# gorgonia/agogo

Hardware: AMD Instinct MI355X
Metric: mcts_sims_per_sec (higher is better)
Workload: dtype f32 (Winograd F(5x5,3x3): fp32 transforms; transform-domain products as fp16x2 = each fp32 operand scaled by a power of two and split into 2 fp16 pieces (22-23 significand bits, absolute error <= 2^-38 of the tensor range), 3 fp16 MFMAs per product, fp32 accumulate)

## Files before the change

agogo_amd/capi.py:

```python
import ctypes as C
import os

import numpy as np

_HERE = os.path.dirname(os.path.abspath(__file__))
_LIB = None

NONE, BLACK, WHITE = 0, 1, 2
PASS, RESIGN = -1, -2
NO_MOVE = -32768
GAME_MNK, GAME_C4, GAME_KOMI, GAME_WQ = 0, 1, 2, 3
ENC_TWOPLANE, ENC_WQ = 0, 1
INF_NET, INF_DUMMY, INF_SCRIPT, INF_HASH, INF_UNIFORM, INF_CALLBACK = 0, 1, 2, 3, 4, 5
BN_DEGENERATE_EPS, BN_RUNNING, BN_IDENTITY = 0, 1, 2
COMPUTE_F32_MFMA, COMPUTE_BF16X3, COMPUTE_FP16X2, COMPUTE_WINO, COMPUTE_AUTO, COMPUTE_WINO_H2 = 0, 1, 2, 3, 4, 5
COMPUTE_FORCE = 0x100
PROF_CONV, PROF_HEADS, PROF_SELECT, PROF_EXPAND, PROF_MOVE, PROF_CONV_INIT = 0, 1, 2, 3, 4, 5
PROF_WINO_IN, PROF_WINO_GEMM, PROF_WINO_OUT = 6, 7, 8
DONT_PREFER_PASS, PREFER_PASS, DONT_RESIGN = 0, 1, 2
POOL_STRICT, POOL_STOP_SEARCH, POOL_GROW = 0, 1, 2


class AgzError(RuntimeError):
    pass
# ... 59 lines not shown

    def tramp(_user, bp):
        try:
            b = bp.contents
            n, F, H, W, pl = b.n, b.features, b.height, b.width, b.policy_len
            as_np = np.ctypeslib.as_array
            leaves = {"planes": as_np(b.planes, shape=(n, F, H, W)), "board": as_np(b.board, shape=(n, H * W)),
                      "to_move": as_np(b.to_move, shape=(n,)), "move_number": as_np(b.move_number, shape=(n,)),
                      "game": as_np(b.game, shape=(n,)), "policy_len": pl}
            pol, val = py(leaves)
            as_np(b.policy, shape=(n, pl))[...] = np.asarray(pol, np.float32).reshape(n, pl)
            as_np(b.value, shape=(n,))[...] = np.asarray(val, np.float32).reshape(n)
            return 0
        except BaseException as e:
            box["exc"] = e
            return 1

    fn = INFER_FN(tramp)
    fn._box = box
    return fn


def lib_path():
    return os.environ.get("AGZ_LIB_PATH") or os.path.join(_HERE, "lib", "libagz.so")


def lib():
    global _LIB
    if _LIB is not None:
        return _LIB
    path = lib_path()
    if not os.path.exists(path):
        raise AgzError("libagz.so not built (%s): run `make` or __graft_entry__.build(); there is no CPU fallback"
                       % path)
    L = C.CDLL(path)
    vp, i32, u64, f64 = C.c_void_p, C.c_int, C.c_uint64, C.c_double
    pvp = C.POINTER(C.c_void_p)
    pf, pi, pu, pu8 = C.POINTER(C.c_float), C.POINTER(C.c_int32), C.POINTER(C.c_uint32), C.POINTER(C.c_uint8)

    def sig(name, res, *args):
        f = getattr(L, name)
        f.restype = res
        f.argtypes = list(args)

    sig("agz_last_error", C.c_char_p)
    sig("agz_version", C.c_char_p)
    sig("agz_ctx_create", i32, i32, pvp)
    sig("agz_ctx_destroy", None, vp)
    sig("agz_ctx_sync", i32, vp)
    sig("agz_ctx_stream", vp, vp)
    sig("agz_ctx_prof_enable", i32, vp, i32)
    sig("agz_ctx_prof_read", i32, vp, i32, C.POINTER(C.c_int64), C.POINTER(C.c_double))
    sig("agz_net_create", i32, vp, C.POINTER(NetConf), pvp)
    sig("agz_net_destroy", None, vp)
    sig("agz_net_num_params", i32, vp)
    sig("agz_net_param_info", i32, vp, i32, C.c_char_p, C.c_size_t, C.POINTER(C.c_size_t))
    sig("agz_net_set_param", i32, vp, i32, pf, C.c_size_t)
    sig("agz_net_get_param", i32, vp, i32, pf, C.c_size_t)
    sig("agz_net_set_bn_stats", i32, vp, i32, pf, pf, C.c_size_t)
    sig("agz_net_init_random", i32, vp, u64)
    sig("agz_net_commit", i32, vp)
    sig("agz_net_infer", i32, vp, pf, i32, pf, pf)
    sig("agz_net_infer_dev", i32, vp, vp, i32, vp, vp)
    sig("agz_host_alloc", i32, vp, C.c_size_t, pvp)
    sig("agz_host_free", i32, vp, vp)
    sig("agz_mcts_to_dot", i32, vp, i32, C.c_char_p, C.c_size_t, C.POINTER(C.c_size_t))
    sig("agz_mcts_set_timeout_ms", i32, vp, i32)
    sig("agz_mcts_last_simulations", i32, vp, C.POINTER(C.c_int64))
    sig("agz_net_set_latency_mode", i32, vp, i32)
    sig("agz_net_set_tower_queues", i32, vp, i32)
    sig("agz_net_set_compute_mode", i32, vp, i32)
    sig("agz_net_flops_per_eval", f64, vp)
    sig("agz_net_save", i32, vp, C.c_char_p)
    sig("agz_net_load", i32, vp, C.c_char_p)
    sig("agz_arena_get_results", i32, vp, C.POINTER(C.c_int64), C.POINTER(C.c_int64), C.POINTER(C.c_int64))
    sig("agz_trainer_create", i32, vp, C.POINTER(NetConf), pvp)
    sig("agz_trainer_create_tied", i32, vp, C.POINTER(NetConf), pvp)
    sig("agz_trainer_is_tied", i32, vp, C.POINTER(i32))
    sig("agz_trainer_destroy", None, vp)
    sig("agz_trainer_num_params", i32, vp)
    sig("agz_trainer_param_info", i32, vp, i32, C.c_char_p, C.c_size_t, C.POINTER(C.c_size_t))
    sig("agz_trainer_set_param", i32, vp, i32, pf, C.c_size_t)
    sig("agz_trainer_get_param", i32, vp, i32, pf, C.c_size_t)
    sig("agz_trainer_get_grad", i32, vp, i32, pf, C.c_size_t)
    sig("agz_trainer_init_random", i32, vp, u64)
    sig("agz_trainer_batch", i32, vp, pf, pf, pf, C.c_float, pf)
    sig("agz_trainer_forward_backward", i32, vp, pf, pf, pf, pf)
    sig("agz_trainer_forward_backward_dev", i32, vp, vp, vp, vp, pf)
    sig("agz_trainer_apply", i32, vp, C.c_float, C.c_float)
    sig("agz_trainer_grads_dev", i32, vp, pvp, C.POINTER(C.c_size_t))
    sig("agz_trainer_set_solver", i32, vp, C.POINTER(SolverConf))
    sig("agz_trainer_get_solver", i32, vp, C.POINTER(SolverConf))
    sig("agz_trainer_get_velocity", i32, vp, i32, pf, C.c_size_t)
    sig("agz_trainer_set_velocity", i32, vp, i32, pf, C.c_size_t)
    sig("agz_trainer_reset_solver", i32, vp)
    sig("agz_trainer_set_adam", i32, vp, C.POINTER(AdamConf))
    sig("agz_trainer_get_adam", i32, vp, C.POINTER(AdamConf), C.POINTER(C.c_uint64))
    sig("agz_trainer_get_moments", i32, vp, i32, pf, pf, C.c_size_t)
    sig("agz_trainer_set_moments", i32, vp, i32, pf, pf, C.c_size_t)
    sig("agz_trainer_set_bn_tracking", i32, vp, i32, C.c_float)
    sig("agz_trainer_get_bn_tracking", i32, vp, C.POINTER(C.c_int), C.POINTER(C.c_float), C.POINTER(C.c_double))
    sig("agz_trainer_num_bn", i32, vp)
    sig("agz_trainer_get_bn_stats", i32, vp, i32, pf, pf, C.c_size_t)
    sig("agz_trainer_set_bn_stats", i32, vp, i32, pf, pf, C.c_size_t, C.c_double)
    sig("agz_trainer_reset_bn_stats", i32, vp)
    sig("agz_trainer_eval", i32, vp, pf, pf, pf, pf)
    sig("agz_trainer_eval_dev", i32, vp, vp, vp, vp, pf)
    sig("agz_trainer_set_compute_mode", i32, vp, i32)
    sig("agz_train", i32, vp, pf, pf, pf, i32, i32, u64, pf)
    sig("agz_trainer_export", i32, vp, vp)
    sig("agz_trainer_save", i32, vp, C.c_char_p)
    sig("agz_trainer_load", i32, vp, C.c_char_p)
    sig("agz_arena_create", i32, vp, C.POINTER(GameConf), C.POINTER(MctsConf), i32, u64, i32, pvp)
    sig("agz_arena_destroy", None, vp)
    sig("agz_arena_set_inferencer", i32, vp, i32, i32, vp)
    sig("agz_arena_reset", i32, vp, pu8)
    sig("agz_arena_play", i32, vp, i32, i32)
    sig("agz_arena_selfplay", i32, vp, C.c_int64, i32)
    sig("agz_arena_set_parallel", i32, vp, i32)
    sig("agz_arena_begin_move", i32, vp)
    sig("agz_arena_simulate", i32, vp, i32)
    sig("agz_arena_end_move", i32, vp, i32)
    sig("agz_arena_apply_moves", i32, vp, pi)
    sig("agz_arena_get_stats", i32, vp, C.POINTER(ArenaStats))
    sig("agz_arena_get_game", i32, vp, i32, pi, C.POINTER(GameState))
    sig("agz_arena_get_history", i32, vp, i32, pi, i32, pi)
    sig("agz_arena_root_children", i32, vp, i32, i32, pi, pu, pf, pf, i32, pi)
    sig("agz_arena_tree_nodes", i32, vp, i32, i32, pi)
    sig("agz_arena_get_examples", i32, vp, pf, pf, pf, pi, i32, pi)
    sig("agz_arena_clear_examples", i32, vp)
    sig("agz_arena_drop_labelled_examples", i32, vp)
    sig("agz_arena_examples_dev", i32, vp, pvp, pvp, pvp, pi)
    i64, pi64 = C.c_int64, C.POINTER(C.c_int64)
    sig("agz_train_dev", i32, vp, vp, vp, vp, i32, i32, u64, pf)
    sig("agz_examples_create", i32, vp, i32, i32, i32, i32, pvp)
    sig("agz_examples_destroy", None, vp)
    sig("agz_examples_count", i32, vp, pi64)
    sig("agz_examples_clear", i32, vp)
    sig("agz_examples_append_arena", i32, vp, vp)
    sig("agz_examples_append_dev", i32, vp, vp, vp, vp, i64)
    sig("agz_examples_append_host", i32, vp, pf, pf, pf, i64)
    sig("agz_examples_get", i32, vp, pf, pf, pf, i64, pi64)
    sig("agz_examples_augment_rotate", i32, vp)
    sig("agz_examples_prepare", i32, vp, i32, i32, u64, pi)
    sig("agz_examples_tensors_dev", i32, vp, pvp, pvp, pvp, pi64, pi)
    sig("agz_examples_get_tensors", i32, vp, pf, pf, pf)
    sig("agz_examples_raw_dev", i32, vp, pvp, pvp, pvp)
    sig("agz_rotate_boards", i32, vp, pf, i32, i32, i32, pf)
    sig("agz_ctx_prof_set_stride", i32, vp, i32, i32)
    sig("agz_wino_stages", i32, vp, pf, pf, i32, i32, i32, i32, i32, pf, pf)
    sig("agz_wino_h2_tile", i32, i32, i32)
    sig("agz_net_set_wino_h2_form", i32, vp, i32)
    sig("agz_net_set_wino_h2_gemm", i32, vp, i32)
    sig("agz_net_min_same_batch", i32, vp, i32, i32, C.POINTER(C.c_int))
    sig("agz_arena_set_prep_compact", i32, vp, i32)
    sig("agz_arena_set_split", i32, vp, i32)
    sig("agz_arena_split_steps", i32, vp, C.POINTER(C.c_int64), C.POINTER(C.c_int64), C.POINTER(C.c_int))
    sig("agz_trainer_set_dma_forward", i32, vp, i32)
    sig("agz_arena_last_prep_batch", i32, vp, C.POINTER(C.c_int), C.POINTER(C.c_int))
    sig("agz_arena_debug_counter", i32, vp, i32, C.POINTER(C.c_int64))
    sig("agz_arena_pool_capacity", i32, vp, C.POINTER(C.c_int), C.POINTER(C.c_int))
    sig("agz_wino_h2_chained", i32, i32, i32, i32)
    sig("agz_arena_random_moves", i32, vp, pi, u64)
    sig("agz_arena_set_state", i32, vp, i32, C.POINTER(State))
    sig("agz_arena_examples_labelled_dev", i32, vp, pvp)
    sig("agz_mcts_create", i32, vp, C.POINTER(GameConf), C.POINTER(MctsConf), u64, i32, pvp)
    sig("agz_mcts_destroy", None, vp)
    sig("agz_mcts_set_inferencer", i32, vp, i32, vp)
    sig("agz_mcts_set_inferencer_callback", i32, vp, INFER_FN, vp, i32)
    sig("agz_arena_set_inferencer_callback", i32, vp, i32, INFER_FN, vp, i32)
    sig("agz_arena_set_pool_policy", i32, vp, i32)
    sig("agz_mcts_set_pool_policy", i32, vp, i32)
    sig("agz_mcts_set_parallel", i32, vp, i32)
    sig("agz_mcts_set_game", i32, vp, C.POINTER(State))
    sig("agz_mcts_search", i32, vp, i32, pi)
    sig("agz_mcts_policies", i32, vp, pf, i32)
    sig("agz_mcts_root_children", i32, vp, pi, pu, pf, pf, i32, pi)
    sig("agz_mcts_nodes", i32, vp, pi)
    sig("agz_mcts_children", i32, vp, i32, pi, pi, pu, pf, pf, i32, pi)
    sig("agz_mcts_get_stats", i32, vp, C.POINTER(ArenaStats))
    sig("agz_mcts_reset", i32, vp)
    sig("agz_comm_init_all", i32, pvp, i32, pvp)
    sig("agz_comm_unique_id", i32, vp)
    sig("agz_comm_init_rank", i32, vp, i32, i32, vp, pvp)
    sig("agz_comm_destroy", None, vp)
    sig("agz_comm_rank", i32, vp)
    sig("agz_comm_size", i32, vp)
    sig("agz_examples_allgather", i32, vp, vp)
    sig("agz_trainer_allreduce", i32, vp, vp)
    sig("agz_trainer_forward_backward_allreduce", i32, vp, vp, pf, pf, pf, pf)
    sig("agz_trainer_forward_backward_allreduce_dev", i32, vp, vp, vp, vp, vp, pf)
    sig("agz_comm_debug_fail_slice", i32, vp, i32)
    sig("agz_trainer_create_sharded", i32, vp, C.POINTER(NetConf), pvp)
    sig("agz_trainer_create_sharded_tied", i32, vp, C.POINTER(NetConf), pvp)
    sig("agz_trainer_shard", i32, vp, C.POINTER(i32), C.POINTER(i32), C.POINTER(i32))
    sig("agz_comm_debug_fail_layer", i32, vp, i32)
    _LIB = L
    return L


def _check(r, what=""):
    if r != 0:
        raise AgzError("%s failed (%d): %s" % (what, r, lib().agz_last_error().decode(errors="replace")))


def _pf(a):
    return a.ctypes.data_as(C.POINTER(C.c_float))


def _pi(a):
    return a.ctypes.data_as(C.POINTER(C.c_int32))


class Ctx:
    def __init__(self, device=0):
        self.h = C.c_void_p()
        self._children = []
        _check(lib().agz_ctx_create(device, C.byref(self.h)), "agz_ctx_create")

    def _adopt(self, child):
        import weakref
        self._children.append(weakref.ref(child))

    def close(self):
        if self.h:
            kids = [r() for r in self._children]
            for k in sorted([k for k in kids if k is not None], key=lambda k: 0 if isinstance(k, Arena) else 1):
                k.close()
            self._children = []
            for p in list(getattr(self, "_pinned", {}).values()):
                lib().agz_host_free(self.h, C.c_void_p(p))
            self._pinned = {}
            lib().agz_ctx_destroy(self.h)
            self.h = C.c_void_p()

    def __del__(self):
        try:
            self.close()
        except Exception:
            pass

    def host_array(self, shape, dtype=np.float32):
        n = int(np.prod(shape)) * np.dtype(dtype).itemsize
        p = C.c_void_p()
        _check(lib().agz_host_alloc(self.h, max(n, 1), C.byref(p)), "agz_host_alloc")
        arr = np.ctypeslib.as_array((C.c_char * max(n, 1)).from_address(p.value)).view(dtype)[: int(np.prod(shape))].reshape(shape)
        self._pinned = getattr(self, "_pinned", {})
        self._pinned[arr.ctypes.data] = p.value
        return arr

    def host_free(self, arr):
        p = getattr(self, "_pinned", {}).pop(arr.ctypes.data, None)
        if p is not None and self.h:
            _check(lib().agz_host_free(self.h, C.c_void_p(p)), "agz_host_free")

    def sync(self):
        _check(lib().agz_ctx_sync(self.h), "agz_ctx_sync")

    def stream(self):
        return lib().agz_ctx_stream(self.h)

    def prof_enable(self, on=True, classes=None):
        if on and classes is not None:
            mask = 0
            for k in classes:
                mask |= 1 << (k + 1)
            _check(lib().agz_ctx_prof_enable(self.h, mask), "agz_ctx_prof_enable")
            return
        return self._prof_enable_all(on)

    def prof_set_stride(self, klass, stride):
        _check(lib().agz_ctx_prof_set_stride(self.h, int(klass), int(stride)), "agz_ctx_prof_set_stride")

    def _prof_enable_all(self, on=True):
        _check(lib().agz_ctx_prof_enable(self.h, int(on)), "agz_ctx_prof_enable")

    def prof_read(self, klass):
        n, ms = C.c_int64(0), C.c_double(0)
        _check(lib().agz_ctx_prof_read(self.h, klass, C.byref(n), C.byref(ms)), "agz_ctx_prof_read")
        return n.value, ms.value


class Net:

    def __init__(self, ctx, K, SharedLayers, FC, Width, Height, Features, ActionSpace, BatchSize=256,
                 bn_mode=BN_DEGENERATE_EPS, bn_eps=1e-5):
        self.ctx = ctx
        self.conf = NetConf(K, SharedLayers, FC, BatchSize, Width, Height, Features, ActionSpace, bn_mode, bn_eps)
        self.h = C.c_void_p()
        _check(lib().agz_net_create(ctx.h, C.byref(self.conf), C.byref(self.h)), "agz_net_create")
        ctx._adopt(self)

    def close(self):
        if self.h and self.ctx.h:
            lib().agz_net_destroy(self.h)
        self.h = C.c_void_p()

    def __del__(self):
        try:
            self.close()
        except Exception:
            pass

    def num_params(self):
        return lib().agz_net_num_params(self.h)

    def param_info(self, i):
        name = C.create_string_buffer(128)
        n = C.c_size_t(0)
        _check(lib().agz_net_param_info(self.h, i, name, 128, C.byref(n)), "agz_net_param_info")
        return name.value.decode(), n.value

    def set_param(self, i, v):
        a = np.ascontiguousarray(v, dtype=np.float32).ravel()
        _check(lib().agz_net_set_param(self.h, i, _pf(a), a.size), "agz_net_set_param")

    def get_param(self, i):
        _, n = self.param_info(i)
        a = np.zeros(n, dtype=np.float32)
        _check(lib().agz_net_get_param(self.h, i, _pf(a), a.size), "agz_net_get_param")
        return a

    def set_bn_stats(self, bi, mean, var):
        m = np.ascontiguousarray(mean, dtype=np.float32)
        v = np.ascontiguousarray(var, dtype=np.float32)
        _check(lib().agz_net_set_bn_stats(self.h, bi, _pf(m), _pf(v), m.size), "agz_net_set_bn_stats")

    def init_random(self, seed):
        _check(lib().agz_net_init_random(self.h, seed), "agz_net_init_random")

    def commit(self):
        _check(lib().agz_net_commit(self.h), "agz_net_commit")

    def infer(self, planes):
        c = self.conf
        x = np.ascontiguousarray(planes, dtype=np.float32).reshape(-1, c.Features, c.Height, c.Width)
        B = x.shape[0]
        pol = np.zeros((B, c.ActionSpace), dtype=np.float32)
        val = np.zeros(B, dtype=np.float32)
        _check(lib().agz_net_infer(self.h, _pf(x), B, _pf(pol), _pf(val)), "agz_net_infer")
        return pol, val

    def set_compute_mode(self, mode):
        _check(lib().agz_net_set_compute_mode(self.h, int(mode)), "agz_net_set_compute_mode")

    def set_latency_mode(self, on=True):
        _check(lib().agz_net_set_latency_mode(self.h, int(on)), "agz_net_set_latency_mode")

    def set_tower_queues(self, queues):
        _check(lib().agz_net_set_tower_queues(self.h, int(queues)), "agz_net_set_tower_queues")

    def set_wino_h2_form(self, form):
        _check(lib().agz_net_set_wino_h2_form(self.h, int(form)), "agz_net_set_wino_h2_form")

    def set_wino_h2_gemm(self, variant):
        _check(lib().agz_net_set_wino_h2_gemm(self.h, int(variant)), "agz_net_set_wino_h2_gemm")

    def min_same_batch(self, n, G):
        b = C.c_int(0)
        _check(lib().agz_net_min_same_batch(self.h, int(n), int(G), C.byref(b)), "agz_net_min_same_batch")
        return b.value

    def infer_dev(self, planes_ptr, B, policy_ptr, value_ptr):
        _check(lib().agz_net_infer_dev(self.h, C.c_void_p(planes_ptr), B, C.c_void_p(policy_ptr),
                                       C.c_void_p(value_ptr)), "agz_net_infer_dev")

    def flops_per_eval(self):
        return lib().agz_net_flops_per_eval(self.h)

    def save(self, path):
        _check(lib().agz_net_save(self.h, os.fsencode(path)), "agz_net_save")

    def load(self, path):
        _check(lib().agz_net_load(self.h, os.fsencode(path)), "agz_net_load")


class Trainer:

    def __init__(self, ctx, K, SharedLayers, FC, Width, Height, Features, ActionSpace, BatchSize, bn_eps=1e-5, tied=False):
        self.ctx = ctx
        self.conf = NetConf(K, SharedLayers, FC, BatchSize, Width, Height, Features, ActionSpace, 0, bn_eps)
        self.h = C.c_void_p()
        if tied:
            _check(lib().agz_trainer_create_tied(ctx.h, C.byref(self.conf), C.byref(self.h)), "agz_trainer_create_tied")
        else:
            _check(lib().agz_trainer_create(ctx.h, C.byref(self.conf), C.byref(self.h)), "agz_trainer_create")
        ctx._adopt(self)

    def is_tied(self):
        v = C.c_int(0)
        _check(lib().agz_trainer_is_tied(self.h, C.byref(v)), "agz_trainer_is_tied")
        return bool(v.value)

    @classmethod
    def sharded(cls, ctx, comm, K, SharedLayers, FC, Width, Height, Features, ActionSpace, BatchSize, bn_eps=1e-5, tied=False):
        assert comm.ctx is ctx, "the communicator belongs to another context"
        self = cls.__new__(cls)
        self.ctx, self.comm = ctx, comm
        self.conf = NetConf(K, SharedLayers, FC, BatchSize, Width, Height, Features, ActionSpace, 0, bn_eps)
        self.h = C.c_void_p()
        if tied:
            _check(lib().agz_trainer_create_sharded_tied(comm.h, C.byref(self.conf), C.byref(self.h)), "agz_trainer_create_sharded_tied")
        else:
            _check(lib().agz_trainer_create_sharded(comm.h, C.byref(self.conf), C.byref(self.h)), "agz_trainer_create_sharded")
        ctx._adopt(self)
        return self

    def shard(self):
        r0, n, nr = C.c_int(0), C.c_int(0), C.c_int(0)
        _check(lib().agz_trainer_shard(self.h, C.byref(r0), C.byref(n), C.byref(nr)), "agz_trainer_shard")
        return r0.value, n.value, nr.value

    def close(self):
        if self.h and self.ctx.h:
            lib().agz_trainer_destroy(self.h)
        self.h = C.c_void_p()

    def __del__(self):
        try:
            self.close()
        except Exception:
            pass

    def num_params(self):
        return lib().agz_trainer_num_params(self.h)

    def param_info(self, i):
        name = C.create_string_buffer(128)
        n = C.c_size_t(0)
        _check(lib().agz_trainer_param_info(self.h, i, name, 128, C.byref(n)), "agz_trainer_param_info")
        return name.value.decode(), n.value

    def set_param(self, i, v):
        a = np.ascontiguousarray(v, dtype=np.float32).ravel()
        _check(lib().agz_trainer_set_param(self.h, i, _pf(a), a.size), "agz_trainer_set_param")

    def get_param(self, i):
        a = np.zeros(self.param_info(i)[1], np.float32)
        _check(lib().agz_trainer_get_param(self.h, i, _pf(a), a.size), "agz_trainer_get_param")
        return a

    def get_grad(self, i):
        a = np.zeros(self.param_info(i)[1], np.float32)
        _check(lib().agz_trainer_get_grad(self.h, i, _pf(a), a.size), "agz_trainer_get_grad")
        return a

    def init_random(self, seed):
        _check(lib().agz_trainer_init_random(self.h, seed), "agz_trainer_init_random")

    def batch(self, planes, pi, v, lr=0.1):
        x = np.ascontiguousarray(planes, np.float32)
        p = np.ascontiguousarray(pi, np.float32)
        vv = np.ascontiguousarray(v, np.float32)
        c = C.c_float(0)
        _check(lib().agz_trainer_batch(self.h, _pf(x), _pf(p), _pf(vv), lr, C.byref(c)), "agz_trainer_batch")
        return c.value

    def forward_backward(self, planes, pi, v):
        x = np.ascontiguousarray(planes, np.float32)
        p = np.ascontiguousarray(pi, np.float32)
        vv = np.ascontiguousarray(v, np.float32)
        c = C.c_float(0)
        _check(lib().agz_trainer_forward_backward(self.h, _pf(x), _pf(p), _pf(vv), C.byref(c)), "agz_trainer_forward_backward")
        return c.value

    def forward_backward_dev(self, planes_ptr, pi_ptr, v_ptr, want_cost=True):
        c = C.c_float(0)
        _check(lib().agz_trainer_forward_backward_dev(self.h, C.c_void_p(planes_ptr), C.c_void_p(pi_ptr), C.c_void_p(v_ptr),
                                                      C.byref(c) if want_cost else None), "agz_trainer_forward_backward_dev")
        return c.value if want_cost else None

    def apply(self, lr=0.1, grad_scale=1.0):
        _check(lib().agz_trainer_apply(self.h, lr, grad_scale), "agz_trainer_apply")

    def set_solver(self, momentum=0.0, l2reg=0.0, clip=0.0, reserved=0):
        sc = SolverConf(momentum, l2reg, clip, reserved)
        _check(lib().agz_trainer_set_solver(self.h, C.byref(sc)), "agz_trainer_set_solver")

    def get_solver(self):
        sc = SolverConf()
        _check(lib().agz_trainer_get_solver(self.h, C.byref(sc)), "agz_trainer_get_solver")
        return {"momentum": sc.momentum, "l2reg": sc.l2reg, "clip": sc.clip}

    def get_velocity(self, i):
        a = np.zeros(self.param_info(i)[1], np.float32)
        _check(lib().agz_trainer_get_velocity(self.h, i, _pf(a), a.size), "agz_trainer_get_velocity")
        return a

    def set_velocity(self, i, v):
        a = np.ascontiguousarray(v, dtype=np.float32).ravel()
        _check(lib().agz_trainer_set_velocity(self.h, i, _pf(a), a.size), "agz_trainer_set_velocity")

    def reset_solver(self):
        _check(lib().agz_trainer_reset_solver(self.h), "agz_trainer_reset_solver")

    def set_adam(self, beta1=0.9, beta2=0.999, eps=1e-8, on=True):
        ac = AdamConf(beta1, beta2, eps, int(on))
        _check(lib().agz_trainer_set_adam(self.h, C.byref(ac)), "agz_trainer_set_adam")

    def get_adam(self):
        ac, t = AdamConf(), C.c_uint64(0)
        _check(lib().agz_trainer_get_adam(self.h, C.byref(ac), C.byref(t)), "agz_trainer_get_adam")
        return {"beta1": ac.beta1, "beta2": ac.beta2, "eps": ac.eps, "on": bool(ac.on), "t": int(t.value)}

    def get_moments(self, i):
        m = np.zeros(self.param_info(i)[1], np.float32)
        v = np.zeros_like(m)
        _check(lib().agz_trainer_get_moments(self.h, i, _pf(m), _pf(v), m.size), "agz_trainer_get_moments")
        return m, v

# ... 561 lines not shown
```

agogo_amd/csrc/conv_wino_h2.hpp:

```cpp
#pragma once

template <int TM> struct WinoT;
template <> struct WinoT<4> {
  static constexpr int AL = 6, VSHIFT = 7;
  static constexpr float BT[6][6] = {{4, 0, -5, 0, 1, 0}, {0, -4, -4, 1, 1, 0}, {0, 4, -4, -1, 1, 0}, {0, -2, -1, 2, 1, 0}, {0, 2, -1, -2, 1, 0}, {0, 4, 0, -5, 0, 1}};
  static constexpr float AT[4][6] = {{1, 1, 1, 1, 1, 0}, {0, 1, -1, 2, -2, 0}, {0, 1, 1, 4, 4, 0}, {0, 1, -1, 8, -8, 1}};
  static constexpr double G[6][3] = {{1.0 / 4, 0, 0}, {-1.0 / 6, -1.0 / 6, -1.0 / 6}, {-1.0 / 6, 1.0 / 6, -1.0 / 6}, {1.0 / 24, 1.0 / 12, 1.0 / 6}, {1.0 / 24, -1.0 / 12, 1.0 / 6}, {0, 0, 1}};
};
template <> struct WinoT<5> {
  static constexpr int AL = 7, VSHIFT = 6;
  static constexpr float BT[7][7] = {{-0.5f, 0.25f, 2.5f, -1.25f, -2, 1, 0}, {0, 0.5f, 0.25f, -2.25f, -1, 1, 0}, {0, -0.5f, 0.75f, 1.75f, -3, 1, 0},
                                     {0, 1, 1.5f, -2, -1.5f, 1, 0},          {0, -1, 2.5f, 0, -2.5f, 1, 0},       {0, 0.25f, 0, -1.25f, 0, 1, 0},
                                     {0, -0.5f, 0.25f, 2.5f, -1.25f, -2, 1}};
  static constexpr float AT[5][7] = {{1, 1, 1, 1, 1, 1, 0}, {0, 1, -1, 0.5f, -0.5f, 2, 0}, {0, 1, 1, 0.25f, 0.25f, 4, 0}, {0, 1, -1, 0.125f, -0.125f, 8, 0},
                                     {0, 1, 1, 0.0625f, 0.0625f, 16, 1}};
  static constexpr double G[7][3] = {{-2, 0, 0}, {-2.0 / 3, -2.0 / 3, -2.0 / 3}, {-2.0 / 9, 2.0 / 9, -2.0 / 9}, {16.0 / 9, 8.0 / 9, 4.0 / 9}, {16.0 / 15, -8.0 / 15, 4.0 / 15},
                                     {2.0 / 45, 4.0 / 45, 8.0 / 45}, {0, 0, 1}};
};
template <int TM> __device__ __forceinline__ void wino_btv(const float* d, float* o);
template <int TM> __device__ __forceinline__ void wino_atv(const float* m, float* o);
template <> __device__ __forceinline__ void wino_btv<4>(const float* d, float* o) { wino_bt6(d, o); }
template <> __device__ __forceinline__ void wino_atv<4>(const float* m, float* o) { wino_at4(m, o); }
template <> __device__ __forceinline__ void wino_btv<5>(const float* d, float* o) {
  o[0] = -0.5f * d[0] + 0.25f * d[1] + 2.5f * d[2] - 1.25f * d[3] - 2.f * d[4] + d[5];
  o[1] = 0.5f * d[1] + 0.25f * d[2] - 2.25f * d[3] - d[4] + d[5];
  o[2] = -0.5f * d[1] + 0.75f * d[2] + 1.75f * d[3] - 3.f * d[4] + d[5];
  o[3] = d[1] + 1.5f * d[2] - 2.f * d[3] - 1.5f * d[4] + d[5];
  o[4] = -d[1] + 2.5f * (d[2] - d[4]) + d[5];
  o[5] = 0.25f * d[1] - 1.25f * d[3] + d[5];
  o[6] = -0.5f * d[1] + 0.25f * d[2] + 2.5f * d[3] - 1.25f * d[4] - 2.f * d[5] + d[6];
}
template <> __device__ __forceinline__ void wino_atv<5>(const float* m, float* o) {
  const float s12 = m[1] + m[2], d12 = m[1] - m[2], s34 = m[3] + m[4], d34 = m[3] - m[4];
  o[0] = m[0] + s12 + s34 + m[5];
  o[1] = d12 + 0.5f * d34 + 2.f * m[5];
  o[2] = s12 + 0.25f * s34 + 4.f * m[5];
  o[3] = d12 + 0.125f * d34 + 8.f * m[5];
  o[4] = s12 + 0.0625f * s34 + 16.f * m[5] + m[6];
}

typedef unsigned u32x2_t __attribute__((ext_vector_type(2)));
struct WinoH2Args;
__device__ __forceinline__ size_t h2_row(const WinoH2Args& h, int pos, int t);
struct WinoH2Args {
  WinoArgs w;
  int tm, npos;
  int rsh, rmask;
  unsigned rA, rB;
  int raw;
  const float* w_unscale_dev;
  int fuse_prev;
  int wm_per_board;
  unsigned* amax_self;
  int in_swap;
  const _Float16* U2;
  const unsigned* amax_in;
  unsigned* amax_out;
  float* wave_max;
  float w_unscale;
  const float* t_in;
  const float* col_unscale;
  const float* t_next;
  int cform;
  const _Float16* U2c;
  const float* amax_true;
  const float* wm_prev;
  float* wm_out;
  unsigned* amax_next;
  float g1, g0;
  int gemm_variant;
  int temporal_stores;
  int row_pad;
};
__device__ __forceinline__ size_t h2_row(const WinoH2Args& h, int pos, int t) {
  return (size_t)(t >> h.rsh) * h.rA + (size_t)pos * h.rB + (size_t)(t & h.rmask);
}

__device__ __forceinline__ void wino_h2_scales(unsigned amax_bits, int shift, float* s, float* inv) {
  int e = (int)((amax_bits >> 23) & 0xffu);
  if (amax_bits == 0u) { *s = 1.f; *inv = 1.f; return; }
  e = e < 30 ? 30 : (e > 230 ? 230 : e);
  *s = __uint_as_float((unsigned)(268 - shift - e) << 23);
  *inv = __uint_as_float((unsigned)(e - 14 + shift) << 23);
}

__device__ __forceinline__ unsigned wino_h2_pack(float a, float b, unsigned* lo) {
  const _Float16 ha = (_Float16)a, hb = (_Float16)b;
  const _Float16 la = (_Float16)(a - (float)ha), lb = (_Float16)(b - (float)hb);
  *lo = (unsigned)__builtin_bit_cast(unsigned short, la) | ((unsigned)__builtin_bit_cast(unsigned short, lb) << 16);
  return (unsigned)__builtin_bit_cast(unsigned short, ha) | ((unsigned)__builtin_bit_cast(unsigned short, hb) << 16);
}

template <int TM>
__global__ __launch_bounds__(256) void wino_in_h2_kernel(WinoH2Args h) {
  using WT = WinoT<TM>;
  constexpr int AL = WT::AL;
  const WinoArgs& a = h.w;
  const int C2 = a.C >> 1;
  const size_t g = (size_t)blockIdx.x * 256 + threadIdx.x;
  if (g >= (size_t)a.T * C2) return;
  const int c2 = (int)(g % C2);
  const int t = (int)(g / C2);
  const int b = t / a.TPB, tt = t - b * a.TPB;
  const int ty = tt / a.ntx, tx = tt - ty * a.ntx;
  unsigned amax_bits;
  if (h.fuse_prev) {
    const float* wp = h.wave_max + (size_t)b * h.wm_per_board;
    float mx = 0.f;
    for (int i = threadIdx.x & 63; i < h.wm_per_board; i += 64) mx = fmaxf(mx, wp[i]);
#pragma unroll
    for (int o = 32; o > 0; o >>= 1) mx = fmaxf(mx, __shfl_xor(mx, o, 64));
    amax_bits = __float_as_uint(mx);
    if (tt == 0 && c2 == 0) h.amax_self[b] = amax_bits;
  } else {
    amax_bits = h.amax_in[b];
  }
  float sb, inv_;
  wino_h2_scales(amax_bits, WT::VSHIFT, &sb, &inv_);
  float sbx = sb, sby = sb;
  if (h.t_in) { const float2 t2 = *reinterpret_cast<const float2*>(h.t_in + 2 * c2); sbx *= t2.x; sby *= t2.y; }
  const float* xb = a.x + (size_t)b * a.Hp * a.Wp * a.C + 2 * c2;
  float2 d[AL][AL];
#pragma unroll
  for (int j = 0; j < AL; j++) {
    const int px = TM * tx + j, pxc = px < a.Wp ? px : a.Wp - 1;
#pragma unroll
    for (int i = 0; i < AL; i++) {
      const int py = TM * ty + i, pyc = py < a.Hp ? py : a.Hp - 1;
      d[i][j] = *reinterpret_cast<const float2*>(xb + ((size_t)pyc * a.Wp + pxc) * a.C);
    }
  }
  float tmx[AL][AL], tmy[AL][AL];
#pragma unroll
  for (int j = 0; j < AL; j++) {
    const bool okx = TM * tx + j < a.Wp;
    float dx[AL], dy[AL], ox[AL], oy[AL];
#pragma unroll
    for (int i = 0; i < AL; i++) {
      const bool ok = okx && TM * ty + i < a.Hp;
      dx[i] = ok ? d[i][j].x : 0.f; dy[i] = ok ? d[i][j].y : 0.f;
    }
    wino_btv<TM>(dx, ox);
    wino_btv<TM>(dy, oy);
#pragma unroll
    for (int i = 0; i < AL; i++) { tmx[i][j] = ox[i]; tmy[i][j] = oy[i]; }
  }
  unsigned* V2 = reinterpret_cast<unsigned*>(a.V);
  const int c = 2 * c2;
  const size_t word_in_row = (size_t)(c >> 5) * 32 + ((c & 31) >> 1);
  const int lane = threadIdx.x & 63;
  const size_t swap_word = (size_t)((c2 >> 6) * 4) * 32 + lane;
#pragma unroll
  for (int i = 0; i < AL; i++) {
    float ox[AL], oy[AL];
    wino_btv<TM>(tmx[i], ox);
    wino_btv<TM>(tmy[i], oy);
#pragma unroll
    for (int j = 0; j < AL; j++) {
      unsigned lo;
      const unsigned hi = wino_h2_pack(ox[j] * sbx, oy[j] * sby, &lo);
      if (h.cform) {
        const auto s16 = __builtin_amdgcn_permlane16_swap(hi, lo, false, false);
        const unsigned e0 = s16[0], e1 = s16[1];
        const int NS = a.C >> 5;
        const size_t chunk0 = ((size_t)(t >> 7) * h.npos + (size_t)(i * AL + j)) * NS + (size_t)((c2 >> 6) * 4 + 2 * (lane >> 5));
        unsigned* p0 = V2 + chunk0 * 4096 + (size_t)(t & 127) * 32 + (lane & 31);
        p0[0] = e0;
        p0[4096] = e1;
        continue;
      }
      unsigned* rowp = V2 + h2_row(h, i * AL + j, t) * a.C;
      if (h.in_swap) {
        const auto s16 = __builtin_amdgcn_permlane16_swap(hi, lo, false, false);
        const unsigned e0 = s16[0], e1 = s16[1];
        const auto s32 = __builtin_amdgcn_permlane32_swap(e0, e1, false, false);
        const unsigned w0 = s32[0], w1 = s32[1];
        rowp[swap_word] = w0;
        rowp[swap_word + 64] = w1;
      } else {
        rowp[word_in_row] = hi;
        rowp[word_in_row + 16] = lo;
      }
    }
  }
}

__global__ __launch_bounds__(256, 3) void wino_gemm_h2_kernel(WinoH2Args h) {
  const WinoArgs& a = h.w;
  constexpr int PIECE = 128 * 64;
  constexpr int STAGE = 4 * PIECE;
  __shared__ __attribute__((aligned(16))) unsigned char lds[STAGE];

  const int per_pos = a.n_mtiles * a.n_ntiles;
  const int nblk = h.npos * per_pos;
  const int id = blockIdx.x;
  int q = nblk >> 3, rr = nblk & 7, xcd = id & 7, slot = id >> 3;
  int tile = (xcd < rr ? xcd * (q + 1) : rr * (q + 1) + (xcd - rr) * q) + slot;
  const int pos = tile / per_pos;
  const int rem = tile - pos * per_pos;
  const int m_tile = rem / a.n_ntiles, n_tile = rem - m_tile * a.n_ntiles;
  const int m0 = m_tile * 128, n0 = n_tile * 128;

  const int tid = threadIdx.x, lane = tid & 63, wid = tid >> 6;
  const int wm = wid >> 1, wn = wid & 1;
  const int srow = tid >> 1, shalf = tid & 1;
  int mrow = m0 + srow;
  if (mrow >= a.T) mrow = a.T - 1;
  int nrow = n0 + srow;
  if (nrow >= a.Ntot) nrow = a.Ntot - 1;
  const int NK = a.C >> 5;
  const unsigned piece_bytes = (unsigned)a.Ntot * 64u;
  unsigned xo_ = (unsigned)((h2_row(h, pos, mrow) * a.C) * 4) + (unsigned)shalf * 32u;
  unsigned wo_ = (unsigned)pos * (unsigned)NK * 2u * piece_bytes + (unsigned)nrow * 64u + (unsigned)shalf * 32u;
  const unsigned s_off0 = h2_lds_off(srow, 2 * shalf), s_off1 = h2_lds_off(srow, 2 * shalf + 1);

  f32x16 acc[2][2];
#pragma unroll
  for (int i = 0; i < 2; i++)
#pragma unroll
    for (int j = 0; j < 2; j++)
#pragma unroll
      for (int r = 0; r < 16; r++) acc[i][j][r] = 0.f;

  int ra[2], rb[2];
#pragma unroll
  for (int i = 0; i < 2; i++) ra[i] = (wm * 2 + i) * 32 + (lane & 31);
#pragma unroll
  for (int j = 0; j < 2; j++) rb[j] = (wn * 2 + j) * 32 + (lane & 31);
  const int kh = lane >> 5;

  u32x4_t xa0, xa1, xa2, xa3, xb0, xb1, xb2, xb3;
  const char* xbase = reinterpret_cast<const char*>(a.V);
  const char* wbase = reinterpret_cast<const char*>(h.U2);
  int f_n = 0;
#define WH2_GLOAD()                                                                           \
  xa0 = *reinterpret_cast<const u32x4_t*>(xbase + xo_);                                       \
  xa1 = *reinterpret_cast<const u32x4_t*>(xbase + xo_ + 16u);                                 \
  xa2 = *reinterpret_cast<const u32x4_t*>(xbase + xo_ + 64u);                                 \
  xa3 = *reinterpret_cast<const u32x4_t*>(xbase + xo_ + 80u);                                 \
  xb0 = *reinterpret_cast<const u32x4_t*>(wbase + wo_);                                       \
  xb1 = *reinterpret_cast<const u32x4_t*>(wbase + wo_ + 16u);                                 \
  xb2 = *reinterpret_cast<const u32x4_t*>(wbase + wo_ + piece_bytes);                         \
  xb3 = *reinterpret_cast<const u32x4_t*>(wbase + wo_ + piece_bytes + 16u);                   \
  if (f_n + 1 < NK) { f_n++; xo_ += 128u; wo_ += 2u * piece_bytes; }
#define WH2_STORE()                                                                           \
  *reinterpret_cast<u32x4_t*>(lds + 0 * PIECE + s_off0) = xa0;                                \
  *reinterpret_cast<u32x4_t*>(lds + 0 * PIECE + s_off1) = xa1;                                \
  *reinterpret_cast<u32x4_t*>(lds + 1 * PIECE + s_off0) = xa2;                                \
  *reinterpret_cast<u32x4_t*>(lds + 1 * PIECE + s_off1) = xa3;                                \
  *reinterpret_cast<u32x4_t*>(lds + 2 * PIECE + s_off0) = xb0;                                \
  *reinterpret_cast<u32x4_t*>(lds + 2 * PIECE + s_off1) = xb1;                                \
  *reinterpret_cast<u32x4_t*>(lds + 3 * PIECE + s_off0) = xb2;                                \
  *reinterpret_cast<u32x4_t*>(lds + 3 * PIECE + s_off1) = xb3;
#define WH2_QUAD(PA_, PB_)                                                                    \
  _Pragma("unroll") for (int i = 0; i < 2; i++)                                               \
    _Pragma("unroll") for (int j = 0; j < 2; j++)                                             \
      acc[i][j] = __builtin_amdgcn_mfma_f32_32x32x16_f16(A_[i][PA_], B_[j][PB_], acc[i][j], 0, 0, 0);

  WH2_GLOAD()
  for (int it = 0; it < NK; it++) {
    WH2_STORE()
    __syncthreads();
    WH2_GLOAD()
#pragma unroll
    for (int ks = 0; ks < 2; ks++) {
      f16x8_t A_[2][2], B_[2][2];
#pragma unroll
      for (int p = 0; p < 2; p++) {
#pragma unroll
        for (int i = 0; i < 2; i++) A_[i][p] = *reinterpret_cast<const f16x8_t*>(lds + p * PIECE + h2_lds_off(ra[i], 2 * ks + kh));
#pragma unroll
        for (int j = 0; j < 2; j++) B_[j][p] = *reinterpret_cast<const f16x8_t*>(lds + (2 + p) * PIECE + h2_lds_off(rb[j], 2 * ks + kh));
      }
      WH2_QUAD(1, 0) WH2_QUAD(0, 1) WH2_QUAD(0, 0)
    }
    __syncthreads();
  }
#undef WH2_QUAD
#undef WH2_STORE
#undef WH2_GLOAD

#pragma unroll
  for (int i = 0; i < 2; i++) {
#pragma unroll
    for (int r = 0; r < 16; r++) {
      const int row = (wm * 2 + i) * 32 + (r & 3) + 8 * (r >> 2) + 4 * (lane >> 5);
      const int m = m0 + row;
      if (m < a.T) {
        float* dst = a.Mb + h2_row(h, pos, m) * a.Ntot;
#pragma unroll
        for (int j = 0; j < 2; j++) {
          const int c = n0 + (wn * 2 + j) * 32 + (lane & 31);
          if (c < a.Ntot) dst[c] = acc[i][j][r];
        }
      }
    }
  }
}

__global__ __launch_bounds__(256, 2) void wino_gemm_h2w_kernel(WinoH2Args h) {
  const WinoArgs& a = h.w;
  constexpr int PA = 128 * 64, PB = 256 * 64;
  constexpr int STAGE = 2 * PA + 2 * PB;
  __shared__ __attribute__((aligned(16))) unsigned char lds[STAGE];

  const int n_nt = (a.Ntot + 255) / 256;
  const int per_pos = a.n_mtiles * n_nt;
  const int nblk = h.npos * per_pos;
  const int id = blockIdx.x;
  int q = nblk >> 3, rr = nblk & 7, xcd = id & 7, slot = id >> 3;
  int tile = (xcd < rr ? xcd * (q + 1) : rr * (q + 1) + (xcd - rr) * q) + slot;
  const int pos = tile / per_pos;
  const int rem = tile - pos * per_pos;
  const int m_tile = rem / n_nt, n_tile = rem - m_tile * n_nt;
  const int m0 = m_tile * 128, n0 = n_tile * 256;

  const int tid = threadIdx.x, lane = tid & 63, wid = tid >> 6;
  const int wm = wid >> 1, wn = wid & 1;
  const int srow = tid >> 1, shalf = tid & 1;
// ... 832 lines not shown
```

agogo_amd/csrc/conv_wino_h2c.hpp:

```cpp
#pragma once

__device__ __forceinline__ unsigned h2c_img(int row, int slot) { return maps::h2c_img(row, slot); }

template <int NK, int PFA>
__global__ __launch_bounds__(256, 2) void wino_gemm_h2c_kernel(WinoH2Args h) {
  const WinoArgs& a = h.w;
  constexpr int SA = 128 * 128, SB = 256 * 128;
  __shared__ __attribute__((aligned(16))) unsigned char lds[SA + SB];

  const int n_nt = a.Ntot >> 8;
  const int per_pos = a.n_mtiles * n_nt;
  const int nblk = h.npos * per_pos;
  const int id = blockIdx.x;
  int q = nblk >> 3, rr = nblk & 7, xcd = id & 7, slot = id >> 3;
  int tile = (xcd < rr ? xcd * (q + 1) : rr * (q + 1) + (xcd - rr) * q) + slot;
  const int pos = tile / per_pos;
  const int rem = tile - pos * per_pos;
  const int m_tile = rem / n_nt, n_tile = rem - m_tile * n_nt;

  const int tid = threadIdx.x, lane = tid & 63, wid = tid >> 6;
  const int wm = wid >> 1, wn = wid & 1;
  const unsigned st_lds = h2c_img(tid >> 3, tid & 7);
  const char* abase = reinterpret_cast<const char*>(a.V) + ((size_t)m_tile * h.npos + pos) * (size_t)NK * SA + (size_t)tid * 16;
  const char* bbase = reinterpret_cast<const char*>(h.U2c) + (((size_t)pos * NK) * n_nt + n_tile) * (size_t)SB + (size_t)tid * 16;
  const size_t bstep = (size_t)n_nt * SB;

  f32x16 acc[2][4];
#pragma unroll
  for (int i = 0; i < 2; i++)
#pragma unroll
    for (int j = 0; j < 4; j++)
#pragma unroll
      for (int r = 0; r < 16; r++) acc[i][j][r] = 0.f;

  const int kh = lane >> 5, sw = (lane >> 1) & 7;
  const unsigned fa = (unsigned)((wm * 64 + (lane & 31)) * 128);
  const unsigned fb = (unsigned)(SA + (wn * 128 + (lane & 31)) * 128);

  u32x4_t xa[PFA][4], xb[8];
  auto load_a = [&](int set, int kk) {
#pragma unroll
    for (int j = 0; j < 4; j++) xa[set][j] = *reinterpret_cast<const u32x4_t*>(abase + (size_t)kk * SA + j * 4096);
  };
  auto load_b = [&](int kk) {
#pragma unroll
    for (int j = 0; j < 8; j++) xb[j] = *reinterpret_cast<const u32x4_t*>(bbase + (size_t)kk * bstep + j * 4096);
  };
  load_b(0);
#pragma unroll
  for (int p = 0; p < PFA; p++) load_a(p, p < NK ? p : NK - 1);
#pragma unroll
  for (int it = 0; it < NK; it++) {
    const int set = it % PFA;
#pragma unroll
    for (int j = 0; j < 4; j++) *reinterpret_cast<u32x4_t*>(lds + st_lds + j * 4096) = xa[set][j];
#pragma unroll
    for (int j = 0; j < 8; j++) *reinterpret_cast<u32x4_t*>(lds + SA + st_lds + j * 4096) = xb[j];
    __syncthreads();
    if (it + 1 < NK) load_b(it + 1);
    if (it + PFA < NK) load_a(set, it + PFA);
#pragma unroll
    for (int ks = 0; ks < 2; ks++) {
      f16x8_t A_[2][2], B_[4][2];
#pragma unroll
      for (int p = 0; p < 2; p++) {
        const unsigned so = (unsigned)(((p * 4 + 2 * ks + kh) ^ sw) << 4);
#pragma unroll
        for (int i = 0; i < 2; i++) A_[i][p] = *reinterpret_cast<const f16x8_t*>(lds + fa + i * 4096 + so);
#pragma unroll
        for (int j = 0; j < 4; j++) B_[j][p] = *reinterpret_cast<const f16x8_t*>(lds + fb + j * 4096 + so);
      }
#pragma unroll
      for (int pp = 0; pp < 3; pp++) {
        const int pa = pp == 0 ? 1 : 0, pb = pp == 1 ? 1 : 0;
#pragma unroll
        for (int i = 0; i < 2; i++)
#pragma unroll
          for (int j = 0; j < 4; j++) acc[i][j] = __builtin_amdgcn_mfma_f32_32x32x16_f16(A_[i][pa], B_[j][pb], acc[i][j], 0, 0, 0);
      }
    }
    __syncthreads();
  }

  float* mbase = a.Mb + ((((size_t)m_tile * h.npos + pos) * (size_t)(a.Ntot >> 6) + (size_t)n_tile * 4 + wn * 2) * 128 + (size_t)(wm * 64)) * 64 + lane;
#pragma unroll
  for (int qq = 0; qq < 2; qq++)
#pragma unroll
    for (int i = 0; i < 2; i++)
#pragma unroll
      for (int r = 0; r < 16; r++) {
        const unsigned x0 = __float_as_uint(acc[i][2 * qq][r]), x1 = __float_as_uint(acc[i][2 * qq + 1][r]);
        const auto s32 = __builtin_amdgcn_permlane32_swap(x0, x1, false, false);
        const unsigned w0 = s32[0], w1 = s32[1];
        float* d = mbase + (size_t)qq * 8192 + (size_t)(i * 32 + (r & 3) + 8 * (r >> 2)) * 64;
        d[0] = __uint_as_float(w0);
        d[4 * 64] = __uint_as_float(w1);
      }
}

typedef __attribute__((address_space(3))) void* h2c_lds_ptr_t;
template <int NK, bool NT = true>
__global__ __launch_bounds__(256, 3) void wino_gemm_h2g_kernel(WinoH2Args h) {
  const WinoArgs& a = h.w;
  constexpr int SA = 128 * 128, SB = 256 * 128;
  __shared__ __attribute__((aligned(16))) unsigned char lds[SA + SB];

  const int n_nt = a.Ntot >> 8;
  const int per_pos = a.n_mtiles * n_nt;
  const int nblk = h.npos * per_pos;
  const int id = blockIdx.x;
  int q = nblk >> 3, rr = nblk & 7, xcd = id & 7, slot = id >> 3;
  int tile = (xcd < rr ? xcd * (q + 1) : rr * (q + 1) + (xcd - rr) * q) + slot;
  const int pos = tile / per_pos;
  const int rem = tile - pos * per_pos;
  const int m_tile = rem / n_nt, n_tile = rem - m_tile * n_nt;

  const int tid = threadIdx.x, lane = tid & 63;
  const int wid = __builtin_amdgcn_readfirstlane(tid >> 6);
  const int wm = wid >> 1, wn = wid & 1;
  const __amdgpu_buffer_rsrc_t ar = h2_rsrc(a.V), br = h2_rsrc(h.U2c);
  const unsigned vo_e = maps::h2c_dma_src(lane, 0), vo_o = maps::h2c_dma_src(lane, 1);
  const unsigned a_w = maps::h2c_wave_part(wid, 128), b_w = maps::h2c_wave_part(wid, 256);
  unsigned a_so = (unsigned)(((size_t)m_tile * h.npos + pos) * (size_t)NK * SA) + a_w;
  unsigned b_so = (unsigned)((((size_t)pos * NK) * n_nt + n_tile) * (size_t)SB) + b_w;
  const unsigned b_step = (unsigned)n_nt * SB;
  unsigned char* const la = lds + a_w;
  unsigned char* const lb = lds + SA + b_w;

  f32x16 acc[2][4];
#pragma unroll
  for (int i = 0; i < 2; i++)
#pragma unroll
    for (int j = 0; j < 4; j++)
#pragma unroll
      for (int r = 0; r < 16; r++) acc[i][j][r] = 0.f;

#pragma nounroll
  for (int it = 0; it < NK; it++) {
#pragma unroll
    for (int j = 0; j < maps::h2c_wave_instrs(128); j++)
      __builtin_amdgcn_raw_ptr_buffer_load_lds(ar, (h2c_lds_ptr_t)(la + maps::h2c_dma_dst(0, j)), 16, (j & 1) ? vo_o : vo_e,
                                               a_so + (maps::h2c_dma_src(0, j) - maps::h2c_dma_src(0, j & 1)), 0, 0);
#pragma unroll
    for (int j = 0; j < maps::h2c_wave_instrs(256); j++)
      __builtin_amdgcn_raw_ptr_buffer_load_lds(br, (h2c_lds_ptr_t)(lb + maps::h2c_dma_dst(0, j)), 16, (j & 1) ? vo_o : vo_e,
                                               b_so + (maps::h2c_dma_src(0, j) - maps::h2c_dma_src(0, j & 1)), 0, 0);
    a_so += SA; b_so += b_step;
    __syncthreads();
#pragma unroll
    for (int ks = 0; ks < 2; ks++) {
      f16x8_t A_[2][2];
#pragma unroll
      for (int i = 0; i < 2; i++) {
        A_[i][0] = *reinterpret_cast<const f16x8_t*>(lds + maps::h2c_frag(wm * 64 + i * 32, lane, 0, ks));
        A_[i][1] = *reinterpret_cast<const f16x8_t*>(lds + maps::h2c_frag(wm * 64 + i * 32, lane, 1, ks));
      }
#pragma unroll
      for (int j = 0; j < 4; j++) {
        const f16x8_t b0 = *reinterpret_cast<const f16x8_t*>(lds + SA + maps::h2c_frag(wn * 128 + j * 32, lane, 0, ks));
        const f16x8_t b1 = *reinterpret_cast<const f16x8_t*>(lds + SA + maps::h2c_frag(wn * 128 + j * 32, lane, 1, ks));
#pragma unroll
        for (int i = 0; i < 2; i++) {
          acc[i][j] = __builtin_amdgcn_mfma_f32_32x32x16_f16(A_[i][1], b0, acc[i][j], 0, 0, 0);
          acc[i][j] = __builtin_amdgcn_mfma_f32_32x32x16_f16(A_[i][0], b1, acc[i][j], 0, 0, 0);
          acc[i][j] = __builtin_amdgcn_mfma_f32_32x32x16_f16(A_[i][0], b0, acc[i][j], 0, 0, 0);
        }
      }
    }
    __syncthreads();
  }

  float* mbase = a.Mb + maps::mc_index(m_tile, h.npos, pos, a.Ntot >> 6, n_tile * 4 + wn * 2, wm * 64, lane);
#pragma unroll
  for (int qq = 0; qq < 2; qq++)
#pragma unroll
    for (int i = 0; i < 2; i++)
#pragma unroll
      for (int r = 0; r < 16; r++) {
        const unsigned x0 = __float_as_uint(acc[i][2 * qq][r]), x1 = __float_as_uint(acc[i][2 * qq + 1][r]);
        const auto s32 = __builtin_amdgcn_permlane32_swap(x0, x1, false, false);
        const unsigned w0 = s32[0], w1 = s32[1];
        float* d = mbase + maps::mc_index(0, 0, 0, 0, qq, i * 32 + maps::mfma_row(r), 0);
        if (NT) {
          __builtin_nontemporal_store(__uint_as_float(w0), d);
          __builtin_nontemporal_store(__uint_as_float(w1), d + maps::mc_index(0, 0, 0, 0, 0, 4, 0));
        } else {
          d[0] = __uint_as_float(w0);
          d[maps::mc_index(0, 0, 0, 0, 0, 4, 0)] = __uint_as_float(w1);
        }
      }
}


typedef unsigned h2p_rsrc_t __attribute__((ext_vector_type(4)));
__device__ __forceinline__ void h2p_dma16(h2p_rsrc_t rsrc, unsigned lds_addr, unsigned voff, unsigned soff) {
  unsigned keep;
  asm volatile("s_mov_b32 %0, m0\n\ts_mov_b32 m0, %1\n\ts_nop 0\n\tbuffer_load_dwordx4 %2, %3, %4 offen lds\n\ts_mov_b32 m0, %0"
               : "=&s"(keep) : "s"(lds_addr), "v"(voff), "s"(rsrc), "s"(soff) : "memory");
}
__device__ __forceinline__ void h2p_dma16x2(h2p_rsrc_t rsrc, unsigned lds_a, unsigned lds_b, unsigned voff_a, unsigned voff_b, unsigned soff) {
  unsigned keep;
  asm volatile("s_mov_b32 %0, m0\n\ts_mov_b32 m0, %1\n\ts_nop 0\n\tbuffer_load_dwordx4 %3, %5, %6 offen lds\n\t"
               "s_mov_b32 m0, %2\n\ts_nop 0\n\tbuffer_load_dwordx4 %4, %5, %6 offen lds\n\ts_mov_b32 m0, %0"
               : "=&s"(keep) : "s"(lds_a), "s"(lds_b), "v"(voff_a), "v"(voff_b), "s"(rsrc), "s"(soff) : "memory");
}
#define H2P_WAIT(N) asm volatile("s_waitcnt vmcnt(%0)" ::"n"(N) : "memory")
template <int MODE>
__global__ __launch_bounds__(256, 1) void wino_gemm_h2p_kernel(WinoH2Args h) {
  const WinoArgs& a = h.w;
  constexpr int NK = maps::H2P_NK, R = maps::H2P_R, SA = 64 * 128, D = maps::H2P_D;
  __shared__ __attribute__((aligned(1024))) unsigned char lds[R * SA];

  const int tid = threadIdx.x, lane = tid & 63;
  const int wid = __builtin_amdgcn_readfirstlane(tid >> 6), wm = wid >> 1, wn = wid & 1;
  const int n_slabs = a.Ntot >> 7, n_nt = a.Ntot >> 8;
  const maps::H2pTeam tm = maps::h2p_team((int)blockIdx.x, (int)gridDim.x, n_slabs);
  if (tm.idle) return;
  const int team = tm.team, slab = tm.slab, nteams = tm.nteams;
  const int n_half = a.n_mtiles * 2, U2 = h.npos * a.n_mtiles;
  const int u0 = maps::h2p_u0(team, nteams, U2), nT = maps::h2p_u0(team + 1, nteams, U2) - u0;
  if (nT <= 0) return;

  h2p_rsrc_t ar;
  {
    const unsigned long long u = (unsigned long long)a.V;
    ar[0] = __builtin_amdgcn_readfirstlane((unsigned)u); ar[1] = __builtin_amdgcn_readfirstlane((unsigned)(u >> 32) & 0xffffu);
    ar[2] = 0x7fffffffu; ar[3] = 0x00020000u;
  }
  const unsigned vo_e = maps::h2c_dma_src(lane, 0), vo_o = maps::h2c_dma_src(lane, 1);
  static_assert(maps::h2c_wave_instrs(64) == 2, "two DMA instructions per wave and stage");
  const unsigned a_w = maps::h2c_wave_part(wid, 64);
  const unsigned dma_l = (unsigned)(size_t)(h2c_lds_ptr_t)lds + a_w;
  auto issue = [&](unsigned vb, int kk, int rslot) {
    if (MODE & 2) return;
    const unsigned so = vb + (unsigned)kk * 16384u + a_w;
    h2p_dma16x2(ar, dma_l + (unsigned)rslot * SA + maps::h2c_dma_dst(0, 0), dma_l + (unsigned)rslot * SA + maps::h2c_dma_dst(0, 1), vo_e, vo_o, so);
  };
  const int kh = lane >> 5;
  auto frag = [&](int rslot, int ks, int p) -> f16x8_t {
    return *reinterpret_cast<const f16x8_t*>(lds + rslot * SA + maps::h2c_frag(wm * 32, lane, p, ks));
  };

  f16x8_t Bf[NK][2][2][2];
  auto load_b = [&](int pos) {
    const char* bb = reinterpret_cast<const char*>(h.U2c) + ((size_t)pos * NK * n_nt + (slab >> 1)) * 32768 +
                     (size_t)(((slab & 1) * 128 + wn * 64 + (lane & 31)) * 128 + kh * 16);
#pragma unroll
    for (int kk = 0; kk < NK; kk++)
#pragma unroll
      for (int ks = 0; ks < 2; ks++)
#pragma unroll
        for (int j = 0; j < 2; j++)
#pragma unroll
          for (int p = 0; p < 2; p++)
            Bf[kk][ks][j][p] = *reinterpret_cast<const f16x8_t*>(bb + (size_t)kk * n_nt * 32768 + j * 4096 + (p * 4 + 2 * ks) * 16);
#pragma unroll
    for (int kk = 0; kk < NK; kk++)
#pragma unroll
      for (int ks = 0; ks < 2; ks++)
#pragma unroll
        for (int j = 0; j < 2; j++)
#pragma unroll
          for (int p = 0; p < 2; p++) asm volatile("" : "+a"(Bf[kk][ks][j][p]));
  };
  auto m_base = [&](int pos, int hm) -> float* {
    return a.Mb + maps::mc_index(hm >> 1, h.npos, pos, a.Ntot >> 6, slab * 2 + wn, (hm & 1) * 64 + wm * 32, lane);
  };
  auto store_rows = [&](const f32x16 (&ac)[2], float* mb, int r) {
    const unsigned x0 = __float_as_uint(ac[0][r]), x1 = __float_as_uint(ac[1][r]);
    const auto s32 = __builtin_amdgcn_permlane32_swap(x0, x1, false, false);
    const unsigned w0 = s32[0], w1 = s32[1];
    float* d = mb + maps::mc_index(0, 0, 0, 0, 0, maps::mfma_row(r), 0);
    if (MODE & 1) { asm volatile("" ::"v"(w0), "v"(w1)); return; }
    __builtin_nontemporal_store(__uint_as_float(w0), d);
    __builtin_nontemporal_store(__uint_as_float(w1), d + maps::mc_index(0, 0, 0, 0, 0, 4, 0));
  };

  int pos = u0 / n_half;
  auto unit_base = [&](int tt) -> unsigned {
    int m = u0 + (tt < nT ? tt : nT - 1) - pos * n_half, p = pos;
    if (m >= n_half) { m -= n_half; p++; }
    return maps::h2p_v_base(p, m, h.npos);
  };
  {
    const unsigned vb0 = unit_base(0), vb1 = unit_base(1);
#pragma unroll
    for (int g = 0; g < D; g++) issue(g < NK ? vb0 : vb1, g % NK, maps::h2p_slot(g / NK, g % NK));
  }
  f32x16 accA[2], accB[2];
#pragma unroll
  for (int j = 0; j < 2; j++)
#pragma unroll
    for (int r = 0; r < 16; r++) accB[j][r] = 0.f;
  f16x8_t Fc[2][2];
  H2P_WAIT(maps::h2p_wait_early() + 2);
  __builtin_amdgcn_s_barrier();
#pragma unroll
  for (int ks = 0; ks < 2; ks++)
#pragma unroll
    for (int p = 0; p < 2; p++) Fc[ks][p] = frag(maps::h2p_slot(0, 0), ks, p);
  float* mprev = m_base(pos, u0 - pos * n_half);

  auto tile = [&](auto par_c, int t, f32x16 (&accC)[2], f32x16 (&accP)[2]) __attribute__((always_inline)) {
    constexpr int PAR = decltype(par_c)::value;
    const int hm = u0 + t - pos * n_half;
    const unsigned vb1 = unit_base(t + 1), vb2 = unit_base(t + 2);
    float* const mcur = m_base(pos, hm);
    const unsigned early = (unsigned)__builtin_amdgcn_readfirstlane((maps::h2p_early(t) || (MODE & 1)) ? 1 : 0);
    f32x16 zero16;
#pragma unroll
    for (int r = 0; r < 16; r++) zero16[r] = 0.f;
#pragma unroll
    for (int kk = 0; kk < NK; kk++) {
      asm volatile("s_cmp_eq_u32 %0, 0\n\ts_cbranch_scc1 .Lh2p_steady_%=\n\ts_waitcnt vmcnt(%1)\n\ts_branch .Lh2p_done_%=\n"
                   ".Lh2p_steady_%=:\n\ts_waitcnt vmcnt(%2)\n.Lh2p_done_%=:" ::"s"(early), "n"(maps::h2p_wait_early()), "n"(maps::h2p_wait_steady()) : "memory", "scc");
      __builtin_amdgcn_s_barrier();
      issue(maps::h2p_tiles_ahead(kk) == 1 ? vb1 : vb2, maps::h2p_kk_ahead(kk), maps::h2p_slot_ahead(PAR, kk));
      f16x8_t Fn[2][2];
#pragma unroll
      for (int ks = 0; ks < 2; ks++)
#pragma unroll
        for (int p = 0; p < 2; p++) Fn[ks][p] = frag(maps::h2p_slot_next(PAR, kk), ks, p);
#pragma unroll
      for (int ks = 0; ks < 2; ks++) {
        accC[0] = __builtin_amdgcn_mfma_f32_32x32x16_f16(Fc[ks][1], Bf[kk][ks][0][0], (kk | ks) ? accC[0] : zero16, 0, 0, 0);
        accC[1] = __builtin_amdgcn_mfma_f32_32x32x16_f16(Fc[ks][1], Bf[kk][ks][1][0], (kk | ks) ? accC[1] : zero16, 0, 0, 0);
        accC[0] = __builtin_amdgcn_mfma_f32_32x32x16_f16(Fc[ks][0], Bf[kk][ks][0][1], accC[0], 0, 0, 0);
        accC[1] = __builtin_amdgcn_mfma_f32_32x32x16_f16(Fc[ks][0], Bf[kk][ks][1][1], accC[1], 0, 0, 0);
        store_rows(accP, mprev, 2 * kk + ks);
        accC[0] = __builtin_amdgcn_mfma_f32_32x32x16_f16(Fc[ks][0], Bf[kk][ks][0][0], accC[0], 0, 0, 0);
        accC[1] = __builtin_amdgcn_mfma_f32_32x32x16_f16(Fc[ks][0], Bf[kk][ks][1][0], accC[1], 0, 0, 0);
      }
#pragma unroll
      for (int ks = 0; ks < 2; ks++)
#pragma unroll
        for (int p = 0; p < 2; p++) Fc[ks][p] = Fn[ks][p];
    }
    mprev = mcur;
  };
  for (int t = 0; t < nT;) {
    const int seg_end = min(nT, (pos + 1) * n_half - u0);
    load_b(pos);
    for (; t < seg_end; t += 2) {
      tile(std::integral_constant<int, 0>{}, t, accA, accB);
      tile(std::integral_constant<int, 1>{}, t + 1, accB, accA);
    }
    pos++;
  }
#pragma unroll
  for (int r = 0; r < 16; r++) store_rows(accB, mprev, r);
  H2P_WAIT(0);
}

template <int TM> __device__ __forceinline__ void wino_at_acc(int nu, float* Y, float t);
template <> __device__ __forceinline__ void wino_at_acc<5>(int nu, float* Y, float t) {
  switch (nu) {
    case 0: Y[0] += t; break;
    case 1: Y[0] += t; Y[1] += t; Y[2] += t; Y[3] += t; Y[4] += t; break;
    case 2: Y[0] += t; Y[1] -= t; Y[2] += t; Y[3] -= t; Y[4] += t; break;
    case 3: Y[0] += t; Y[1] += 0.5f * t; Y[2] += 0.25f * t; Y[3] += 0.125f * t; Y[4] += 0.0625f * t; break;
    case 4: Y[0] += t; Y[1] -= 0.5f * t; Y[2] += 0.25f * t; Y[3] -= 0.125f * t; Y[4] += 0.0625f * t; break;
    case 5: Y[0] += t; Y[1] += 2.f * t; Y[2] += 4.f * t; Y[3] += 8.f * t; Y[4] += 16.f * t; break;
    default: Y[4] += t; break;
  }
}
template <> __device__ __forceinline__ void wino_at_acc<4>(int nu, float* Y, float t) {
  switch (nu) {
    case 0: Y[0] += t; break;
    case 1: Y[0] += t; Y[1] += t; Y[2] += t; Y[3] += t; break;
    case 2: Y[0] += t; Y[1] -= t; Y[2] += t; Y[3] -= t; break;
    case 3: Y[0] += t; Y[1] += 2.f * t; Y[2] += 4.f * t; Y[3] += 8.f * t; break;
    case 4: Y[0] += t; Y[1] -= 2.f * t; Y[2] += 4.f * t; Y[3] -= 8.f * t; break;
    default: Y[3] += t; break;
  }
}

template <int TM, bool LAST>
__global__ __launch_bounds__(256, 2) void wino_oi_h2c_kernel(WinoH2Args h) {
  using WT = WinoT<TM>;
  constexpr int AL = WT::AL;
  const WinoArgs& a = h.w;
  extern __shared__ __attribute__((aligned(16))) float ys[];
  const int tid = threadIdx.x, tl = tid >> 4, pr = tid & 15, lane = tid & 63;
  const int s = blockIdx.y, NS = a.C >> 5, HW = a.H * a.W;
  const int t0 = blockIdx.x * 16;
  const int t = t0 + tl;
  const bool live = t < a.T;
  const int tc = live ? t : a.T - 1;
  const int b = tc / a.TPB, tt = tc - b * a.TPB;
  const int ty = tt / a.ntx, tx = tt - ty * a.ntx;
  const int bl = tl / a.TPB;
  float s_, un0;
  wino_h2_scales(h.amax_in[b], WT::VSHIFT, &s_, &un0);
  const __amdgpu_buffer_rsrc_t mr = h2_rsrc(a.Mb + ((size_t)(t0 >> 7) * h.npos * NS + s) * 8192);
  const unsigned m_lane = (unsigned)(((tc & 127) * 64 + pr * 4) * 4);
  const unsigned m_pos = (unsigned)NS * 32768u;
  float Y[TM][TM][4];
#pragma unroll
  for (int k = 0; k < TM; k++)
#pragma unroll
    for (int l = 0; l < TM; l++)
#pragma unroll
      for (int e = 0; e < 4; e++) Y[k][l][e] = 0.f;
  float4 m[2][AL];
#pragma unroll
  for (int xi = 0; xi < AL; xi++) m[0][xi] = h2_ldf4(mr, m_lane, (unsigned)(xi * AL) * m_pos);
#pragma unroll
  for (int nu = 0; nu < AL; nu++) {
    if (nu + 1 < AL) {
#pragma unroll
      for (int xi = 0; xi < AL; xi++) m[(nu + 1) & 1][xi] = h2_ldf4(mr, m_lane, (unsigned)(xi * AL + nu + 1) * m_pos);
    }
    float mm[4][AL], oo[4][TM];
#pragma unroll
    for (int xi = 0; xi < AL; xi++) { const float4 v = m[nu & 1][xi]; mm[0][xi] = v.x; mm[1][xi] = v.y; mm[2][xi] = v.z; mm[3][xi] = v.w; }
#pragma unroll
    for (int e = 0; e < 4; e++) wino_atv<TM>(mm[e], oo[e]);
#pragma unroll
    for (int k = 0; k < TM; k++)
#pragma unroll
      for (int e = 0; e < 4; e++) {
        float yl[TM];
#pragma unroll
        for (int l = 0; l < TM; l++) yl[l] = Y[k][l][e];
        wino_at_acc<TM>(nu, yl, oo[e][k]);
#pragma unroll
        for (int l = 0; l < TM; l++) Y[k][l][e] = yl[l];
      }
    __builtin_amdgcn_sched_barrier(0);
  }
  const char* ep = reinterpret_cast<const char*>(a.ep);
  const unsigned e_lane = (unsigned)(32 * s + 2 * pr) * 16u, e_pix = (unsigned)a.Cout_p * 16u;
  float mx = 0.f;
  float* yb = LAST ? a.y + (size_t)b * a.Hp * a.Wp * a.Cout_p + 32 * s + 2 * pr : nullptr;
#pragma unroll
  for (int k = 0; k < TM; k++) {
    const int hh = TM * ty + k, hc = hh < a.H ? hh : a.H - 1;
#pragma unroll
    for (int l = 0; l < TM; l++) {
      const int ww = TM * tx + l, wc = ww < a.W ? ww : a.W - 1;
      const char* e = ep + (size_t)(hc * a.W + wc) * e_pix + e_lane;
      const float4 E0 = *reinterpret_cast<const float4*>(e), E1 = *reinterpret_cast<const float4*>(e + 16);
      float va = (Y[k][l][0] * un0) * E0.x + E0.y, vb = (Y[k][l][1] * un0) * E0.z + E0.w;
      float vc = (Y[k][l][2] * un0) * E1.x + E1.y, vd = (Y[k][l][3] * un0) * E1.z + E1.w;
      va = va > 0.f ? va : 0.f; vb = vb > 0.f ? vb : 0.f; vc = vc > 0.f ? vc : 0.f; vd = vd > 0.f ? vd : 0.f;
      const float y0 = va + vb, y1 = vc + vd;
      if (live && hh < a.H && ww < a.W) {
        if (LAST) *reinterpret_cast<float2*>(yb + ((size_t)(hh + 1) * a.Wp + (ww + 1)) * a.Cout_p) = make_float2(y0, y1);
        else *reinterpret_cast<float2*>(&ys[((size_t)bl * HW + hh * a.W + ww) * 32 + 2 * pr]) = make_float2(y0, y1);
        mx = fmaxf(mx, fmaxf(y0, y1));
      }
    }
    __builtin_amdgcn_sched_barrier(0);
  }
  if (LAST) return;
#pragma unroll
  for (int o = 8; o > 0; o >>= 1) mx = fmaxf(mx, __shfl_xor(mx, o, 64));
  if (pr == 0 && live) h.wm_out[(size_t)t * NS + s] = mx;
  float ax;
  if (h.amax_true) ax = __uint_as_float(reinterpret_cast<const unsigned*>(h.amax_true)[b]);
  else {
    const int wmpb = a.TPB * NS;
    const float* wp = h.wm_prev + (size_t)b * wmpb;
    ax = 0.f;
    for (int i = pr; i < wmpb; i += 16) ax = fmaxf(ax, wp[i]);
#pragma unroll
    for (int o = 8; o > 0; o >>= 1) ax = fmaxf(ax, __shfl_xor(ax, o, 64));
  }
  const float bound = h.g1 * ax + h.g0;
  const unsigned bbits = __float_as_uint(bound);
  if (s == 0 && tt == 0 && pr == 0 && live) h.amax_next[b] = bbits;
  float sb, inv_;
  wino_h2_scales(bbits, WT::VSHIFT, &sb, &inv_);
  __syncthreads();
  const float* yl = ys + (size_t)bl * HW * 32 + 2 * pr;
  float tmx[AL][AL], tmy[AL][AL];
#pragma unroll
  for (int j = 0; j < AL; j++) {
    const int ww = TM * tx + j - 1;
    const bool okx = ww >= 0 && ww < a.W;
    const int wc = ww < 0 ? 0 : (ww < a.W ? ww : a.W - 1);
    float dx[AL], dy[AL], ox[AL], oy[AL];
#pragma unroll
    for (int i = 0; i < AL; i++) {
      const int hh = TM * ty + i - 1;
      const bool ok = okx && hh >= 0 && hh < a.H;
      const int hc = hh < 0 ? 0 : (hh < a.H ? hh : a.H - 1);
      const float2 d = *reinterpret_cast<const float2*>(yl + (size_t)(hc * a.W + wc) * 32);
      dx[i] = ok ? d.x : 0.f; dy[i] = ok ? d.y : 0.f;
    }
    wino_btv<TM>(dx, ox);
    wino_btv<TM>(dy, oy);
#pragma unroll
    for (int i = 0; i < AL; i++) { tmx[i][j] = ox[i]; tmy[i][j] = oy[i]; }
  }
  const float sv = live ? sb : 0.f;
  const __amdgpu_buffer_rsrc_t vr = h2_rsrc(reinterpret_cast<const char*>(a.V) + ((size_t)(t0 >> 7) * h.npos * NS + s) * 16384);
  const unsigned v_lane = (unsigned)(((t0 & 127) + (tid >> 6) * 4) * 128 + lane * 4);
  const unsigned v_pos = (unsigned)NS * 16384u;
#pragma unroll
  for (int i = 0; i < AL; i++) {
    float ox[AL], oy[AL];
    wino_btv<TM>(tmx[i], ox);
    wino_btv<TM>(tmy[i], oy);
#pragma unroll
    for (int j = 0; j < AL; j++) {
      unsigned lo;
      const unsigned hi = wino_h2_pack(ox[j] * sv, oy[j] * sv, &lo);
      const auto s16 = __builtin_amdgcn_permlane16_swap(hi, lo, false, false);
      const unsigned e0 = s16[0], e1 = s16[1];
      const auto s32 = __builtin_amdgcn_permlane32_swap(e0, e1, false, false);
      const unsigned w0 = s32[0], w1 = s32[1];
      __builtin_amdgcn_raw_buffer_store_b32(w0, vr, v_lane, (unsigned)(i * AL + j) * v_pos, 0);
      __builtin_amdgcn_raw_buffer_store_b32(w1, vr, v_lane + 256u, (unsigned)(i * AL + j) * v_pos, 0);
    }
  }
}

typedef float f2c __attribute__((ext_vector_type(2)));
template <int TM> __device__ __forceinline__ void wino_atv_p(const f2c* m, f2c* o);
template <> __device__ __forceinline__ void wino_atv_p<4>(const f2c* m, f2c* o) {
  const f2c s12 = m[1] + m[2], d12 = m[1] - m[2], s34 = m[3] + m[4], d34 = m[3] - m[4];
  o[0] = m[0] + s12 + s34;
  o[1] = d12 + 2.f * d34;
  o[2] = s12 + 4.f * s34;
  o[3] = d12 + 8.f * d34 + m[5];
}
template <> __device__ __forceinline__ void wino_atv_p<5>(const f2c* m, f2c* o) {
  const f2c s12 = m[1] + m[2], d12 = m[1] - m[2], s34 = m[3] + m[4], d34 = m[3] - m[4];
  o[0] = m[0] + s12 + s34 + m[5];
  o[1] = d12 + 0.5f * d34 + 2.f * m[5];
  o[2] = s12 + 0.25f * s34 + 4.f * m[5];
  o[3] = d12 + 0.125f * d34 + 8.f * m[5];
  o[4] = s12 + 0.0625f * s34 + 16.f * m[5] + m[6];
}
template <int TM> __device__ __forceinline__ void wino_at_acc_p(int nu, f2c* Y, f2c t);
template <> __device__ __forceinline__ void wino_at_acc_p<5>(int nu, f2c* Y, f2c t) {
  switch (nu) {
    case 0: Y[0] += t; break;
    case 1: Y[0] += t; Y[1] += t; Y[2] += t; Y[3] += t; Y[4] += t; break;
    case 2: Y[0] += t; Y[1] -= t; Y[2] += t; Y[3] -= t; Y[4] += t; break;
    case 3: Y[0] += t; Y[1] += 0.5f * t; Y[2] += 0.25f * t; Y[3] += 0.125f * t; Y[4] += 0.0625f * t; break;
    case 4: Y[0] += t; Y[1] -= 0.5f * t; Y[2] += 0.25f * t; Y[3] -= 0.125f * t; Y[4] += 0.0625f * t; break;
    case 5: Y[0] += t; Y[1] += 2.f * t; Y[2] += 4.f * t; Y[3] += 8.f * t; Y[4] += 16.f * t; break;
    default: Y[4] += t; break;
  }
}
template <> __device__ __forceinline__ void wino_at_acc_p<4>(int nu, f2c* Y, f2c t) {
  switch (nu) {
    case 0: Y[0] += t; break;
    case 1: Y[0] += t; Y[1] += t; Y[2] += t; Y[3] += t; break;
    case 2: Y[0] += t; Y[1] -= t; Y[2] += t; Y[3] -= t; break;
    case 3: Y[0] += t; Y[1] += 2.f * t; Y[2] += 4.f * t; Y[3] += 8.f * t; break;
    case 4: Y[0] += t; Y[1] -= 2.f * t; Y[2] += 4.f * t; Y[3] -= 8.f * t; break;
    default: Y[3] += t; break;
  }
}
template <int TM> __device__ __forceinline__ f2c wino_bt_row_p(int i, const f2c* d);
template <> __device__ __forceinline__ f2c wino_bt_row_p<5>(int i, const f2c* d) {
  switch (i) {
    case 0: return -0.5f * d[0] + 0.25f * d[1] + 2.5f * d[2] - 1.25f * d[3] - 2.f * d[4] + d[5];
    case 1: return 0.5f * d[1] + 0.25f * d[2] - 2.25f * d[3] - d[4] + d[5];
    case 2: return -0.5f * d[1] + 0.75f * d[2] + 1.75f * d[3] - 3.f * d[4] + d[5];
    case 3: return d[1] + 1.5f * d[2] - 2.f * d[3] - 1.5f * d[4] + d[5];
    case 4: return -d[1] + 2.5f * (d[2] - d[4]) + d[5];
    case 5: return 0.25f * d[1] - 1.25f * d[3] + d[5];
    default: return -0.5f * d[1] + 0.25f * d[2] + 2.5f * d[3] - 1.25f * d[4] - 2.f * d[5] + d[6];
  }
}
template <> __device__ __forceinline__ f2c wino_bt_row_p<4>(int i, const f2c* d) {
  switch (i) {
    case 0: return 4.f * d[0] - 5.f * d[2] + d[4];
    case 1: return -4.f * d[1] - 4.f * d[2] + d[3] + d[4];
    case 2: return 4.f * d[1] - 4.f * d[2] - d[3] + d[4];
    case 3: return -2.f * d[1] - d[2] + 2.f * d[3] + d[4];
    case 4: return 2.f * d[1] - d[2] - 2.f * d[3] + d[4];
    default: return 4.f * d[1] - 5.f * d[3] + d[5];
  }
}
template <int TM> __device__ __forceinline__ void wino_btv_p(const f2c* d, f2c* o) {
#pragma unroll
  for (int i = 0; i < TM + 2; i++) o[i] = wino_bt_row_p<TM>(i, d);
}

template <int TM, bool NT = true>
__global__ __launch_bounds__(256, 2) void wino_oip_h2c_kernel(WinoH2Args h) {
  constexpr int MAUX = 0, VAUX = NT ? 2 : 0;
  using WT = WinoT<TM>;
  constexpr int AL = WT::AL, NPRE = AL - 3;
  const WinoArgs& a = h.w;
  extern __shared__ __attribute__((aligned(16))) float ys[];
  const int tid = threadIdx.x, tl = tid >> 4, pr = tid & 15, lane = tid & 63;
  const int NS = a.C >> 5;
  const int PH = TM * a.nty + 2, PW = TM * a.ntx + 2;
  const int bpg = 16 / a.TPB;
  const int n_groups = (a.T + 15) >> 4, n_items = n_groups * NS;
  const int tt = tl % a.TPB, bl = tl / a.TPB;
  const int ty = tt / a.ntx, tx = tt - ty * a.ntx;
  for (int i = tid; i < bpg * PH * PW * 32; i += 256) ys[i] = 0.f;
  const __amdgpu_buffer_rsrc_t mr = h2_rsrc(a.Mb);
  const __amdgpu_buffer_rsrc_t vr = h2_rsrc(a.V);
  const unsigned m_lane = (unsigned)((tl * 64 + pr * 4) * 4);
  const unsigned v_lane = (unsigned)((((tid >> 6) * 4) * 128) + lane * 4);
  const unsigned e_pix = (unsigned)a.Cout_p * 16u;
  float* const ybase = ys + ((size_t)bl * PH * PW + (size_t)(TM * ty) * PW + TM * tx) * 32 + 2 * pr;
  unsigned okmask = 0;
#pragma unroll
  for (int k = 0; k < TM; k++)
#pragma unroll
    for (int l = 0; l < TM; l++) okmask |= (TM * ty + k < a.H && TM * tx + l < a.W) ? 1u << (k * TM + l) : 0u;
  const __amdgpu_buffer_rsrc_t er = h2_rsrc(a.ep);
  float4 m[NPRE][AL];
  auto m_soff = [&](int g, int s, int pos) -> unsigned { return (unsigned)((((g >> 3) * h.npos + pos) * NS + s)) * 32768u + (unsigned)(g & 7) * 4096u; };
  int item = blockIdx.x;
  {
    const int g = __builtin_amdgcn_readfirstlane(item / NS), s = __builtin_amdgcn_readfirstlane(item - (item / NS) * NS);
#pragma unroll
    for (int nu = 0; nu < NPRE; nu++)
#pragma unroll
      for (int xi = 0; xi < AL; xi++) m[nu][xi] = h2_ldf4<MAUX>(mr, m_lane, m_soff(g, s, xi * AL + nu));
  }
  __syncthreads();
  for (; item < n_items; item += gridDim.x) {
    const int g = __builtin_amdgcn_readfirstlane(item / NS), s = __builtin_amdgcn_readfirstlane(item - (item / NS) * NS);
    const int t = g * 16 + tl;
    const bool live = t < a.T;
    const int b = live ? g * bpg + bl : (a.T - 1) / a.TPB;
    float s_, un0;
    wino_h2_scales(h.amax_in[b], WT::VSHIFT, &s_, &un0);
    f2c Y[TM][TM][2];
#pragma unroll
    for (int k = 0; k < TM; k++)
#pragma unroll
      for (int l = 0; l < TM; l++) { Y[k][l][0] = f2c{0.f, 0.f}; Y[k][l][1] = f2c{0.f, 0.f}; }
#pragma unroll
    for (int nu = 0; nu < AL; nu++) {
      f2c c0[AL], c1[AL], o0[TM], o1[TM];
#pragma unroll
      for (int xi = 0; xi < AL; xi++) {
        const float4 v = m[nu % NPRE][xi];
        c0[xi] = f2c{v.x, v.y}; c1[xi] = f2c{v.z, v.w};
      }
      if (nu + NPRE < AL) {
#pragma unroll
        for (int xi = 0; xi < AL; xi++) m[nu % NPRE][xi] = h2_ldf4<MAUX>(mr, m_lane, m_soff(g, s, xi * AL + nu + NPRE));
      }
      wino_atv_p<TM>(c0, o0);
      wino_atv_p<TM>(c1, o1);
#pragma unroll
      for (int k = 0; k < TM; k++) {
        f2c y0[TM], y1[TM];
#pragma unroll
        for (int l = 0; l < TM; l++) { y0[l] = Y[k][l][0]; y1[l] = Y[k][l][1]; }
        wino_at_acc_p<TM>(nu, y0, o0[k]);
        wino_at_acc_p<TM>(nu, y1, o1[k]);
#pragma unroll
        for (int l = 0; l < TM; l++) { Y[k][l][0] = y0[l]; Y[k][l][1] = y1[l]; }
      }
      __builtin_amdgcn_sched_barrier(0);
    }
    __builtin_amdgcn_sched_barrier(0);
    unsigned e_base = (unsigned)(32 * s + 2 * pr) * 16u + (unsigned)((TM * ty) * a.W + TM * tx) * e_pix;
    asm volatile("" : "+v"(e_base));
    float4 E[2][TM][2];
    auto load_e = [&](int buf, int k) {
#pragma unroll
      for (int l = 0; l < TM; l++) {
        const bool ok = (okmask >> (k * TM + l)) & 1u;
        const unsigned off = e_base + (ok ? (unsigned)(k * a.W + l) * e_pix : 0u);
        E[buf][l][0] = h2_ldf4(er, off, 0);
        E[buf][l][1] = h2_ldf4(er, off + 16u, 0);
      }
    };
    load_e(0, 0);
    float mxv = 0.f;
    float* yw = ybase;
    asm volatile("" : "+v"(yw));
#pragma unroll
    for (int k = 0; k < TM; k++) {
      if (k + 1 < TM) load_e((k + 1) & 1, k + 1);
#pragma unroll
      for (int l = 0; l < TM; l++) {
        const bool ok = live && ((okmask >> (k * TM + l)) & 1u);
        const float4 E0 = E[k & 1][l][0], E1 = E[k & 1][l][1];
        const f2c u0 = Y[k][l][0] * un0, u1 = Y[k][l][1] * un0;
        float va = u0.x * E0.x + E0.y, vb = u0.y * E0.z + E0.w;
        float vc = u1.x * E1.x + E1.y, vd = u1.y * E1.z + E1.w;
        va = va > 0.f ? va : 0.f; vb = vb > 0.f ? vb : 0.f; vc = vc > 0.f ? vc : 0.f; vd = vd > 0.f ? vd : 0.f;
        const float y0 = ok ? va + vb : 0.f, y1 = ok ? vc + vd : 0.f;
        *reinterpret_cast<float2*>(yw + ((k + 1) * PW + l + 1) * 32) = make_float2(y0, y1);
        mxv = fmaxf(mxv, fmaxf(y0, y1));
      }
      __builtin_amdgcn_sched_barrier(0);
    }
#pragma unroll
    for (int o = 8; o > 0; o >>= 1) mxv = fmaxf(mxv, __shfl_xor(mxv, o, 64));
    if (pr == 0 && live) h.wm_out[(size_t)t * NS + s] = mxv;
    float ax;
    if (h.amax_true) ax = __uint_as_float(reinterpret_cast<const unsigned*>(h.amax_true)[b]);
    else {
      const int wmpb = a.TPB * NS;
      const float* wp = h.wm_prev + (size_t)b * wmpb;
      ax = 0.f;
      for (int i = pr; i < wmpb; i += 16) ax = fmaxf(ax, wp[i]);
#pragma unroll
      for (int o = 8; o > 0; o >>= 1) ax = fmaxf(ax, __shfl_xor(ax, o, 64));
    }
    const float bound = h.g1 * ax + h.g0;
    const unsigned bbits = __float_as_uint(bound);
    if (s == 0 && tt == 0 && pr == 0 && live) h.amax_next[b] = bbits;
    float sb, inv_;
    wino_h2_scales(bbits, WT::VSHIFT, &sb, &inv_);
    const float sv = live ? sb : 0.f;
    __syncthreads();
    {
      const int nx = item + (int)gridDim.x < n_items ? item + (int)gridDim.x : item;
      const int g2 = __builtin_amdgcn_readfirstlane(nx / NS), s2 = __builtin_amdgcn_readfirstlane(nx - (nx / NS) * NS);
#pragma unroll
      for (int nu = 0; nu < NPRE; nu++)
#pragma unroll
        for (int xi = 0; xi < AL; xi++) m[nu][xi] = h2_ldf4<MAUX>(mr, m_lane, m_soff(g2, s2, xi * AL + nu));
    }
    __builtin_amdgcn_sched_barrier(0);
    const unsigned v_base = (unsigned)((((g >> 3) * h.npos) * NS + s)) * 16384u + (unsigned)(g & 7) * 2048u;
    const unsigned v_pos = (unsigned)NS * 16384u;
    const float* yr = ybase;
    asm volatile("" : "+v"(yr));
#pragma unroll
    for (int i0 = 0; i0 < AL; i0 += 3) {
      constexpr int NRMAX = 3;
      const int nr = AL - i0 < NRMAX ? AL - i0 : NRMAX;
      f2c tmr[NRMAX][AL];
#pragma unroll
      for (int j = 0; j < AL; j++) {
        f2c d[AL];
#pragma unroll
        for (int ii = 0; ii < AL; ii++) {
          const float2 v = *reinterpret_cast<const float2*>(yr + (ii * PW + j) * 32);
          d[ii] = f2c{v.x, v.y};
        }
#pragma unroll
        for (int r = 0; r < NRMAX; r++)
          if (r < nr) tmr[r][j] = wino_bt_row_p<TM>(i0 + r, d);
      }
      __builtin_amdgcn_sched_barrier(0);
#pragma unroll
      for (int r = 0; r < NRMAX; r++) {
        if (r >= nr) continue;
        const int i = i0 + r;
        f2c o[AL];
        wino_btv_p<TM>(tmr[r], o);
#pragma unroll
        for (int j = 0; j < AL; j++) {
          unsigned lo;
          const unsigned hi = wino_h2_pack(o[j].x * sv, o[j].y * sv, &lo);
          const auto s16 = __builtin_amdgcn_permlane16_swap(hi, lo, false, false);
          const unsigned e0 = s16[0], e1 = s16[1];
          const auto s32 = __builtin_amdgcn_permlane32_swap(e0, e1, false, false);
          const unsigned w0 = s32[0], w1 = s32[1];
          __builtin_amdgcn_raw_buffer_store_b32(w0, vr, v_lane, v_base + (unsigned)(i * AL + j) * v_pos, VAUX);
          __builtin_amdgcn_raw_buffer_store_b32(w1, vr, v_lane + 256u, v_base + (unsigned)(i * AL + j) * v_pos, VAUX);
        }
      }
      __builtin_amdgcn_sched_barrier(0);
    }
    __syncthreads();
  }
}

static void wino_build_u2c(const std::vector<_Float16>& u2, std::vector<_Float16>& u2c, int npos, int Ntot, int C, int Cout_p) {
  const int NC = C / 32, NT = Ntot / 256;
  u2c.assign(u2.size(), (_Float16)0.f);
  for (int pos = 0; pos < npos; pos++)
    for (int kc = 0; kc < NC; kc++)
      for (int nn = 0; nn < Ntot; nn++) {
        const int s = nn >> 6, j2 = nn & 63, ch = 32 * s + (j2 >> 1), br = j2 & 1, n = br * Cout_p + ch;
        for (int p = 0; p < 2; p++) {
          const _Float16* src = &u2[((((size_t)pos * NC + kc) * 2 + p) * Ntot + n) * 32];
          _Float16* dst = &u2c[((((size_t)pos * NC + kc) * NT + (nn >> 8)) * 256 + (nn & 255)) * 64 + p * 32];
          for (int k = 0; k < 32; k++) dst[k] = src[k];
        }
      }
}

static inline bool wino_h2c_ok(int H, int W, int tm, int Kp) {
  const int tpb = ceil_div(H, tm) * ceil_div(W, tm);
  const int nk = Kp / 32;
  return Kp % 128 == 0 && 16 % tpb == 0 && (nk == 4 || nk == 8 || nk == 12 || nk == 16) &&
         (size_t)(16 / tpb) * (tm * ceil_div(H, tm) + 2) * (tm * ceil_div(W, tm) + 2) * 128 <= 80 * 1024;
}

static void wino_h2c_geometry(WinoH2Args& h) {
  WinoArgs& a = h.w;
  const int tm = h.tm == 5 ? 5 : 4;
  h.tm = tm; h.npos = (tm + 2) * (tm + 2);
  a.nty = ceil_div(a.H, tm); a.ntx = ceil_div(a.W, tm); a.TPB = a.nty * a.ntx; a.T = a.B * a.TPB;
  h.rsh = 7; h.rmask = 127; h.rA = (unsigned)h.npos * 128u; h.rB = 128u;
  a.n_mtiles = ceil_div(a.T, 128); a.n_ntiles = ceil_div(a.Ntot, 128);
  h.in_swap = 1; h.cform = 1; h.wm_per_board = 0;
}
static void wino_h2c_in(agz_ctx* ctx, WinoH2Args& h, hipStream_t st) {
  wino_h2c_geometry(h);
  h.fuse_prev = 0; h.amax_self = const_cast<unsigned*>(h.amax_in);
  ProfScopeOn ps(ctx, AGZ_PROF_WINO_IN, st == ctx->stream.raw());
  const size_t n_in = (size_t)h.w.T * (h.w.C / 2);
  if (h.tm == 5) hipLaunchKernelGGL(wino_in_h2_kernel<5>, dim3((unsigned)((n_in + 255) / 256)), dim3(256), 0, st, h);
  else hipLaunchKernelGGL(wino_in_h2_kernel<4>, dim3((unsigned)((n_in + 255) / 256)), dim3(256), 0, st, h);
}
constexpr int WINO_H2_GEMM_DEFAULT = 1;
static void wino_h2c_gemm(agz_ctx* ctx, WinoH2Args& h, hipStream_t st) {
  wino_h2c_geometry(h);
  ProfScopeOn ps(ctx, AGZ_PROF_WINO_GEMM, st == ctx->stream.raw());
  const dim3 g(h.npos * h.w.n_mtiles * (h.w.Ntot >> 8));
  const bool dma_ok = wino_h2_rows(h.npos, (size_t)h.w.T) * h.w.C * 4 < ((size_t)1 << 31) && (size_t)h.npos * h.w.C * h.w.Ntot * 4 < ((size_t)1 << 31);
  const int variant_all = h.gemm_variant > 0 ? h.gemm_variant : WINO_H2_GEMM_DEFAULT;
  const int variant = variant_all & 15, mode = (variant_all >> 4) & 3;
  const int n_slabs = h.w.Ntot >> 7;
  if (variant == 2 && dma_ok && (h.w.C >> 5) == 8 && h.w.Ntot % 256 == 0 && ctx->num_cus / 8 >= n_slabs) {
    const dim3 gp((unsigned)(8 * ((ctx->num_cus / 8) / n_slabs) * n_slabs));
    switch (mode) {
      case 1: hipLaunchKernelGGL(wino_gemm_h2p_kernel<1>, gp, dim3(256), 0, st, h); break;
      case 2: hipLaunchKernelGGL(wino_gemm_h2p_kernel<2>, gp, dim3(256), 0, st, h); break;
      case 3: hipLaunchKernelGGL(wino_gemm_h2p_kernel<3>, gp, dim3(256), 0, st, h); break;
      default: hipLaunchKernelGGL(wino_gemm_h2p_kernel<0>, gp, dim3(256), 0, st, h); break;
    }
    return;
  }
  if (dma_ok && h.temporal_stores && (h.w.C >> 5) == 8) { hipLaunchKernelGGL((wino_gemm_h2g_kernel<8, false>), g, dim3(256), 0, st, h); return; }
  if (dma_ok) {
    switch (h.w.C >> 5) {
      case 4: hipLaunchKernelGGL((wino_gemm_h2g_kernel<4>), g, dim3(256), 0, st, h); return;
      case 8: hipLaunchKernelGGL((wino_gemm_h2g_kernel<8>), g, dim3(256), 0, st, h); return;
      case 12: hipLaunchKernelGGL((wino_gemm_h2g_kernel<12>), g, dim3(256), 0, st, h); return;
      default: hipLaunchKernelGGL((wino_gemm_h2g_kernel<16>), g, dim3(256), 0, st, h); return;
    }
  }
  switch (h.w.C >> 5) {
    case 4: hipLaunchKernelGGL((wino_gemm_h2c_kernel<4, 2>), g, dim3(256), 0, st, h); break;
    case 8: hipLaunchKernelGGL((wino_gemm_h2c_kernel<8, 2>), g, dim3(256), 0, st, h); break;
    case 12: hipLaunchKernelGGL((wino_gemm_h2c_kernel<12, 2>), g, dim3(256), 0, st, h); break;
    default: hipLaunchKernelGGL((wino_gemm_h2c_kernel<16, 2>), g, dim3(256), 0, st, h); break;
  }
}
static void wino_h2c_oi(agz_ctx* ctx, WinoH2Args& h, bool last, hipStream_t st, int variant = 4) {
  wino_h2c_geometry(h);
  ProfScopeOn ps(ctx, AGZ_PROF_WINO_OUT, st == ctx->stream.raw());
  const WinoArgs& a = h.w;
  const dim3 g((unsigned)ceil_div(a.T, 16), (unsigned)(a.C >> 5));
  const size_t shm = last ? 0 : (size_t)(16 / a.TPB) * a.H * a.W * 32 * sizeof(float);
  const bool fits31 = wino_h2_rows(h.npos, (size_t)a.T) * a.Ntot * 4 < ((size_t)1 << 31);
  if (variant == 4 && !last && fits31 && !(ctx->func_attr_state & 2u)) {
    const bool ok = hipFuncSetAttribute(reinterpret_cast<const void*>(&wino_oip_h2c_kernel<5>), hipFuncAttributeMaxDynamicSharedMemorySize, 80 * 1024) == hipSuccess &&
                    hipFuncSetAttribute(reinterpret_cast<const void*>(&wino_oip_h2c_kernel<4>), hipFuncAttributeMaxDynamicSharedMemorySize, 80 * 1024) == hipSuccess;
    if (!ok) (void)hipGetLastError();
    ctx->func_attr_state |= 2u | (ok ? 1u : 0u);
  }
  if (variant == 4 && !last && fits31 && (ctx->func_attr_state & 1u)) {
    const size_t shp = (size_t)(16 / a.TPB) * (h.tm * a.nty + 2) * (h.tm * a.ntx + 2) * 32 * sizeof(float);
    const int items = ceil_div(a.T, 16) * (a.C >> 5);
    const dim3 gp((unsigned)std::min(items, 2 * ctx->num_cus));
    if (h.tm == 5 && h.temporal_stores) {
      (void)hipFuncSetAttribute(reinterpret_cast<const void*>(&wino_oip_h2c_kernel<5, false>), hipFuncAttributeMaxDynamicSharedMemorySize, 80 * 1024);
      hipLaunchKernelGGL((wino_oip_h2c_kernel<5, false>), gp, dim3(256), shp, st, h);
      return;
    }
    if (h.tm == 5) hipLaunchKernelGGL((wino_oip_h2c_kernel<5>), gp, dim3(256), shp, st, h);
    else hipLaunchKernelGGL((wino_oip_h2c_kernel<4>), gp, dim3(256), shp, st, h);
    return;
  }
  if (h.tm == 5) {
    if (last) hipLaunchKernelGGL((wino_oi_h2c_kernel<5, true>), g, dim3(256), shm, st, h);
    else hipLaunchKernelGGL((wino_oi_h2c_kernel<5, false>), g, dim3(256), shm, st, h);
  } else {
    if (last) hipLaunchKernelGGL((wino_oi_h2c_kernel<4, true>), g, dim3(256), shm, st, h);
    else hipLaunchKernelGGL((wino_oi_h2c_kernel<4, false>), g, dim3(256), shm, st, h);
  }
}
```

agogo_amd/csrc/gemm_maps.hpp:

```cpp
#pragma once
#include <cstddef>
#if defined(__HIPCC__)
#define AGZ_MAPS_HD __host__ __device__
#else
#define AGZ_MAPS_HD
#endif

namespace agz {
namespace maps {

AGZ_MAPS_HD constexpr unsigned h2c_img(int row, int unit) { return (unsigned)(row * 128 + ((unit ^ ((row >> 1) & 7)) << 4)); }

AGZ_MAPS_HD constexpr unsigned h2c_dma_src(int lane, int j) {
  return (unsigned)(j * 1024 + (lane >> 3) * 128 + (((lane & 7) ^ ((4 * j + (lane >> 4)) & 7)) << 4));
}
AGZ_MAPS_HD constexpr unsigned h2c_dma_dst(int lane, int j) { return (unsigned)(j * 1024 + lane * 16); }
AGZ_MAPS_HD constexpr unsigned h2c_wave_part(int wid, int stage_rows) { return (unsigned)(wid * (stage_rows / 4) * 128); }
AGZ_MAPS_HD constexpr int h2c_wave_instrs(int stage_rows) { return stage_rows / 4 / 8; }

AGZ_MAPS_HD constexpr unsigned h2c_frag(int row0, int lane, int piece, int ks) {
  return (unsigned)((row0 + (lane & 31)) * 128 + (((piece * 4 + 2 * ks + (lane >> 5)) ^ ((lane >> 1) & 7)) << 4));
}

AGZ_MAPS_HD constexpr int mfma_row(int r) { return (r & 3) + 8 * (r >> 2); }

AGZ_MAPS_HD constexpr size_t mc_index(int m_tile, int npos, int pos, int n_slices, int slice, int row, int col) {
  return ((((size_t)m_tile * npos + pos) * (size_t)n_slices + (size_t)slice) * 128 + (size_t)row) * 64 + (size_t)col;
}

constexpr int H2P_D = 10, H2P_R = 16, H2P_NK = 8;
AGZ_MAPS_HD constexpr unsigned h2p_v_base(int pos, int hm, int npos) {
  return (unsigned)(((hm >> 1) * npos + pos) * (H2P_NK * 16384) + (hm & 1) * 8192);
}
AGZ_MAPS_HD constexpr int h2p_slot(int par, int kk) { return (par * H2P_NK + kk) % H2P_R; }
AGZ_MAPS_HD constexpr int h2p_slot_next(int par, int kk) { return (par * H2P_NK + kk + 1) % H2P_R; }
AGZ_MAPS_HD constexpr int h2p_slot_ahead(int par, int kk) { return (par * H2P_NK + kk + H2P_D) % H2P_R; }
AGZ_MAPS_HD constexpr int h2p_kk_ahead(int kk) { return (kk + H2P_D) % H2P_NK; }
AGZ_MAPS_HD constexpr int h2p_tiles_ahead(int kk) { return (kk + H2P_D) / H2P_NK; }
AGZ_MAPS_HD constexpr int h2p_wait_steady() { return 4 + (H2P_D - 2) * 6; }
AGZ_MAPS_HD constexpr int h2p_wait_early() { return (H2P_D - 2) * 2; }
AGZ_MAPS_HD constexpr bool h2p_early(int t) { return t < 2; }
struct H2pTeam { int team, slab, nteams; bool idle; };
AGZ_MAPS_HD constexpr H2pTeam h2p_team(int block, int grid, int n_slabs) {
  const int xcd = block & 7, slot = block >> 3, tpx = (grid >> 3) / n_slabs;
  return H2pTeam{xcd * tpx + (tpx ? slot / n_slabs : 0), tpx ? slot % n_slabs : 0, 8 * tpx, slot >= tpx * n_slabs};
}
AGZ_MAPS_HD constexpr int h2p_u0(int team, int nteams, int U2) { return 2 * (int)((long)team * U2 / nteams); }

}
}
```

agogo_amd/csrc/net.hip:

```cpp
#include "net.hpp"
#include "gemm_maps.hpp"

#include <cmath>
#include <cstdio>
#include <cstring>
#include <type_traits>

typedef float f32x16 __attribute__((ext_vector_type(16)));
typedef float f32x4 __attribute__((ext_vector_type(4)));

namespace agz {

struct ConvArgs {
  const float* x;
  const float* w;
  const void* ep;
  float* y;
  int M, HW, W, Wp, HpWp;
  int Cin_p, Cout_p, Ntot;
  int n_mtiles, n_ntiles;
  int raw;
  int splits;
  int per;
  float* ws;
// ... 947 lines not shown
      for (int n = 0; n < 2 * Kp; n++)
        for (int ci = 0; ci < Kp; ci++)
          for (int tap = 0; tap < 9; tap++) l1s[l][n] += std::fabs(getw(n, ci, tap)) / (double)tin[ci];
    }
    AGZ_HIP_TRY(hipStreamSynchronize(ctx->stream));
    tins[l] = tin; coluns[l] = colun;
  }
  AGZ_REQUIRE((int)h_ep_dual.size() == conf.SharedLayers && !h_ep_init.empty(), AGZ_E_STATE, "agz_net: Winograd weights before commit");
  const int hw = H * W;
  std::vector<float> e2;
  for (int l = 0; l < conf.SharedLayers; l++) {
    const std::vector<float>& e = h_ep_dual[l];
    const bool more = l + 1 < conf.SharedLayers;
    e2.assign(e.size(), 0.f);
    for (int p = 0; p < hw; p++)
      for (int c = 0; c < Kp; c++) {
        const float tn = more ? tins[l + 1][c] : 1.0f;
        const size_t o = ((size_t)p * Kp + c) * 4;
        e2[o + 0] = e[o + 0] * coluns[l][c] * tn; e2[o + 1] = e[o + 1] * tn;
        e2[o + 2] = e[o + 2] * coluns[l][Kp + c] * tn; e2[o + 3] = e[o + 3] * tn;
      }
    if (chained) {
      double g1 = 0.0, g0 = 0.0;
      for (int p = 0; p < hw; p++)
        for (int c = 0; c < Kp; c++) {
          const double tn = more ? tins[l + 1][c] : 1.0;
          const size_t o = ((size_t)p * Kp + c) * 4;
          g1 = std::max(g1, tn * (std::fabs((double)e[o + 0]) * l1s[l][c] + std::fabs((double)e[o + 2]) * l1s[l][Kp + c]));
          g0 = std::max(g0, tn * (std::max((double)e[o + 1], 0.0) + std::max((double)e[o + 3], 0.0)));
        }
      wino_g1[l] = (float)(g1 * (1.0 + 1e-6)); wino_g0[l] = (float)(g0 * (1.0 + 1e-6));
    }
    AGZ_HIP_TRY(hipMalloc(&d_ep_h2[l], e2.size() * 4));
    AGZ_HIP_TRY(hipMemcpyAsync(d_ep_h2[l], e2.data(), e2.size() * 4, hipMemcpyHostToDevice, ctx->stream));
    AGZ_HIP_TRY(hipStreamSynchronize(ctx->stream));
  }
  if (conf.SharedLayers > 0) {
    e2.assign(h_ep_init.size(), 0.f);
    for (int p = 0; p < hw; p++)
      for (int c = 0; c < Kp; c++) {
        const size_t o = ((size_t)p * Kp + c) * 2;
        e2[o] = h_ep_init[o] * tins[0][c]; e2[o + 1] = h_ep_init[o + 1] * tins[0][c];
      }
    AGZ_HIP_TRY(hipMalloc(&d_ep_init_h2, e2.size() * 4));
    AGZ_HIP_TRY(hipMemcpyAsync(d_ep_init_h2, e2.data(), e2.size() * 4, hipMemcpyHostToDevice, ctx->stream));
    AGZ_HIP_TRY(hipStreamSynchronize(ctx->stream));
  }
  return AGZ_OK;
}

agz_net::FwdPlan agz_net::fwd_plan(int B) const {
  const int M = B * HW;
  FwdPlan p{};
  auto n_tiles128 = [&](int ntot) { return ceil_div(M, 128) * ceil_div(ntot, 128); };
  p.half_init = cfg == 0 && n_tiles128(Kp) < ctx->num_cus;
  p.half_dual = cfg == 0 && n_tiles128(2 * Kp) < ctx->num_cus;
  const int tiles_dual = cfg != 0 ? ceil_div(M, 128) * ceil_div(2 * Kp, 64) : ceil_div(M, 64) * ceil_div(2 * Kp, 128);
  p.small = latency_mode && Kp >= 64 &&
            (tiles_dual * 4 <= ctx->num_cus || (Kp >= 256 && tiles_dual <= ctx->num_cus));
  p.forced_split = compute_force && cfg == 0 && conf.SharedLayers > 0 &&
                   (this->compute_mode == AGZ_COMPUTE_WINO_H2 || this->compute_mode == AGZ_COMPUTE_WINO ||
                    this->compute_mode == AGZ_COMPUTE_BF16X3 || this->compute_mode == AGZ_COMPUTE_FP16X2);
  p.latency = p.small && !p.forced_split;
  const int spread_max = 64;
  p.heads_spread = p.small || (latency_mode && (B <= spread_max || Kp >= 256));
  p.heads_nb = B >= 32;
  p.split_ok = cfg == 0 && !p.latency && (!p.half_dual || compute_force) && conf.SharedLayers > 0 &&
               (size_t)B * Hp * Wp * Kp * sizeof(float) < ((size_t)1 << 32);
  {
    const int npos = (wino_tm + 2) * (wino_tm + 2), tpb = ceil_div(H, wino_tm) * ceil_div(W, wino_tm);
    p.wino_wide = (2 * Kp) % 256 == 0 && (size_t)npos * ceil_div(B * tpb, 128) * ((2 * Kp) / 256) >= (size_t)ctx->num_cus;
  }
  return p;
}

int agz_net::min_same_batch(int n, int G) const {
  if (n >= G) return G;
  const FwdPlan want = fwd_plan(G);
  auto same = [&](int B) {
    const FwdPlan q = fwd_plan(B);
    return q.half_init == want.half_init && q.half_dual == want.half_dual && q.small == want.small && q.forced_split == want.forced_split &&
           q.latency == want.latency && q.heads_spread == want.heads_spread && q.split_ok == want.split_ok && q.heads_nb == want.heads_nb && q.wino_wide == want.wino_wide;
  };
  if (same(n)) return n;
  for (int B = 16; B < G; B *= 2)
    if (B > n && same(B)) return B;
  return G;
}

agz_net::H2Tower agz_net::wino_h2_tower(int B) const {
  H2Tower t{};
  t.npos = (wino_tm + 2) * (wino_tm + 2);
  t.tpb = ceil_div(H, wino_tm) * ceil_div(W, wino_tm);
  static const int chunk_env = [] { const char* e = getenv("AGZ_WINO_H2_CHUNK"); return e ? atoi(e) : 0; }();
  static const int queues_env = [] { const char* e = getenv("AGZ_WINO_H2_QUEUES"); return e ? atoi(e) : 0; }();
  const int queues_want = queues_env > 0 ? queues_env : (tower_queues > 0 ? tower_queues : (B >= 256 ? 2 : 1));
  const int chunk_max = (int)std::min<size_t>((size_t)B, ((((size_t)1 << 32) - 1) / ((size_t)t.npos * Kp * 4) - 127) / t.tpb);
  t.chunk = chunk_env >= 1 ? std::min(chunk_env, chunk_max) : chunk_max;
  t.ns = (queues_want == 2 && B >= 64) ? 2 : 1;
  if (t.ns == 2 && t.chunk >= B) t.chunk = (B + 1) / 2;
  t.v_elems = wino_h2_rows(t.npos, (size_t)t.chunk * t.tpb) * Kp; t.m_elems = 2 * t.v_elems;
  static const int form_env = [] { const char* e = getenv("AGZ_WINO_H2_FORM"); return e ? atoi(e) : -1; }();
  t.form_want = wino_form >= 0 ? wino_form : form_env;
  t.chained = t.form_want != 0 && (int)d_u2c_dual.size() == conf.SharedLayers && agz::wino_h2c_ok(H, W, wino_tm, Kp);
  t.n_scr = t.chained ? ceil_div(B, t.chunk) : t.ns;
  t.wm_board = t.chained ? (size_t)t.tpb * (Kp >> 5) * 2 : (size_t)t.tpb * (Kp >> 6);
  return t;
}

int agz_net::wino_h2_reserve(int B, const H2Tower& t, bool* amax_moved) {
  if (t.v_elems * t.n_scr > wino_v_cap) {
    AGZ_HIP_TRY(hipStreamSynchronize(ctx->stream));
    if (ctx->stream2) AGZ_HIP_TRY(hipStreamSynchronize(ctx->stream2));
    if (d_wV) hipFree(d_wV);
    if (d_wM) hipFree(d_wM);
    d_wV = d_wM = nullptr; wino_chunk_cap = 0;
    AGZ_HIP_TRY(hipMalloc(&d_wV, t.v_elems * t.n_scr * sizeof(float)));
    AGZ_HIP_TRY(hipMalloc(&d_wM, t.m_elems * t.n_scr * sizeof(float)));
    wino_v_cap = t.v_elems * t.n_scr; wino_chunk_cap = 0;
  }
  const size_t need_amax = (size_t)(conf.SharedLayers + 1) * B + t.wm_board * B;
  if (need_amax > amax_cap) {
    AGZ_HIP_TRY(hipStreamSynchronize(ctx->stream));
    if (ctx->stream2) AGZ_HIP_TRY(hipStreamSynchronize(ctx->stream2));
    if (d_amax) hipFree(d_amax);
    d_amax = nullptr; amax_cap = 0;
    AGZ_HIP_TRY(hipMalloc(&d_amax, need_amax * sizeof(unsigned)));
    amax_cap = need_amax;
    if (amax_moved) *amax_moved = true;
  }
  return AGZ_OK;
}

void agz_net::wino_h2c_block(int l, int B, int b0, int ci, const H2Tower& t, hipStream_t st, float* cur, float* nxt) {
  const size_t wmb = (size_t)t.tpb * (Kp >> 5);
  const bool last = l + 1 == conf.SharedLayers;
  float* d_wave_max = reinterpret_cast<float*>(d_amax + (size_t)(conf.SharedLayers + 1) * B);
  WinoH2Args hh{};
  WinoArgs& wa = hh.w;
  wa.x = cur + (size_t)b0 * Hp * Wp * Kp; wa.y = nxt + (size_t)b0 * Hp * Wp * Kp;
  wa.V = d_wV + (size_t)ci * t.v_elems; wa.Mb = d_wM + (size_t)ci * t.m_elems; wa.ep = d_ep_h2[l];
  wa.B = std::min(t.chunk, B - b0); wa.H = H; wa.W = W; wa.Hp = Hp; wa.Wp = Wp; wa.C = Kp; wa.Cout_p = Kp; wa.Ntot = 2 * Kp;
  hh.U2c = d_u2c_dual[l]; hh.w_unscale = 1.f; hh.tm = wino_tm;
  hh.amax_in = d_amax + (size_t)l * B + b0;
  hh.amax_next = last ? nullptr : d_amax + (size_t)(l + 1) * B + b0;
  hh.amax_true = l == 0 ? reinterpret_cast<const float*>(d_amax + b0) : nullptr;
  hh.wm_prev = d_wave_max + ((size_t)((l + 1) & 1) * B + b0) * wmb;
  hh.wm_out = d_wave_max + ((size_t)(l & 1) * B + b0) * wmb;
  hh.g1 = wino_g1[l]; hh.g0 = wino_g0[l];
  {
    static const int gemm_env = [] {
      const char* e = getenv("AGZ_WINO_H2_GEMM");
      const int v = e ? atoi(e) : 0;
      if (v == 0 || (((v & 63) == 1 || (v & 63) == 2) && (v >> 6) <= 1)) return v;
      fprintf(stderr, "libagz: AGZ_WINO_H2_GEMM=%s ignored (want 1 or 2, optionally + 64)\n", e);
      return 0;
    }();
    const int gv = wino_gemm > 0 ? wino_gemm : gemm_env;
    hh.gemm_variant = gv & 63; hh.temporal_stores = (gv >> 6) & 1;
  }
  if (l == 0) agz::wino_h2c_in(ctx, hh, st);
  agz::wino_h2c_gemm(ctx, hh, st);
  agz::wino_h2c_oi(ctx, hh, last, st, t.form_want == 1 ? 1 : 4);
}

void agz_net::heads_spread_range(agz::HeadArgs h, bool nb4, int B, int b0, int nb, hipStream_t st) {
  h.x += (size_t)b0 * Hp * Wp * Kp;
  h.feat = d_hs + (size_t)b0 * 3 * HW; h.cols = d_hs + (size_t)B * 3 * HW + (size_t)b0 * (conf.ActionSpace + conf.FC);
  h.policy += (size_t)b0 * conf.ActionSpace; h.value += b0;
  hipLaunchKernelGGL(heads_feat_kernel, dim3(ceil_div(HW, 4), nb), dim3(256), 0, st, h);
  if (nb4)
    hipLaunchKernelGGL(heads_fc_nb_kernel<4>, dim3(ceil_div(conf.ActionSpace + conf.FC, 64), ceil_div(nb, 4)), dim3(1024), 0, st, h, nb);
  else
    hipLaunchKernelGGL(heads_fc_kernel, dim3(ceil_div(conf.ActionSpace + conf.FC, 64), nb), dim3(1024), 0, st, h);
  hipLaunchKernelGGL(heads_out_kernel, dim3(nb), dim3(256), 0, st, h);
}

bool agz_net::half_ok(int B) const {
  if (!committed || B < 2 || B > max_batch || (B & 1) || (B / 2) % 4 != 0 || cfg != 0 || conf.SharedLayers <= 0) return false;
  if (min_same_batch(B / 2, B) != B / 2) return false;
  const FwdPlan plan = fwd_plan(B);
  int mode = compute_mode;
  if (mode == AGZ_COMPUTE_AUTO) mode = !d_u2_dual.empty() ? AGZ_COMPUTE_WINO_H2 : AGZ_COMPUTE_BF16X3;
  if (!plan.split_ok || plan.latency || mode != AGZ_COMPUTE_WINO_H2 || !plan.heads_spread || !plan.heads_nb) return false;
  if ((int)d_u2_dual.size() != conf.SharedLayers || !d_ep_init_h2) return false;
  if (!d_w3_init || Kp % 128 != 0 || (size_t)B * Hp * Wp * Fp * sizeof(float) >= ((size_t)1 << 32)) return false;
  const H2Tower t = wino_h2_tower(B);
  return t.chained && t.ns == 2 && t.chunk * 2 == B;
}

int agz_net::forward_half_reserve(int B) {
  const H2Tower t = wino_h2_tower(B);
  int r = wino_h2_reserve(B, t, nullptr);
  if (r != AGZ_OK) return r;
  const size_t need = (size_t)B * (3 * HW + conf.ActionSpace + conf.FC);
  if (need > hs_cap) {
    AGZ_HIP_TRY(hipStreamSynchronize(ctx->stream));
    if (d_hs) hipFree(d_hs);
    d_hs = nullptr; hs_cap = 0;
    AGZ_HIP_TRY(hipMalloc(&d_hs, need * sizeof(float)));
    hs_cap = need;
  }
  return AGZ_OK;
}

int agz_net::forward_half(int B, int half, hipStream_t st, float* policy_dev, float* value_dev, hipEvent_t mid) {
  const int nb = B / 2, b0 = half * nb;
  const FwdPlan plan = fwd_plan(B);
  const H2Tower t = wino_h2_tower(B);
  ConvArgs a{};
  a.M = nb * HW; a.HW = HW; a.W = W; a.Wp = Wp; a.HpWp = Hp * Wp;
  a.x = d_act_in + (size_t)b0 * Hp * Wp * Fp; a.w = d_w_init; a.ep = d_ep_init_h2; a.y = d_actA + (size_t)b0 * Hp * Wp * Kp;
  a.Cin_p = Fp; a.Cout_p = Kp; a.Ntot = Kp;
  a.n_ntiles = ceil_div(a.Ntot, 128); a.n_mtiles = ceil_div(a.M, 128);
  a.splits = 1; a.per = 0; a.ws = nullptr; a.raw = 0;
  AGZ_HIP_TRY(hipMemsetAsync(d_amax + b0, 0, (size_t)nb * sizeof(unsigned), st));
  a.amax_out = d_amax + b0;
  hipLaunchKernelGGL((conv3x3_x3_kernel<false>), dim3(a.n_mtiles * a.n_ntiles), dim3(256), 0, st, a, d_w3_init);
  const int L = conf.SharedLayers;
  for (int l = 0; l < L; l++) {
    wino_h2c_block(l, B, b0, half, t, st, d_actA, d_actB);
    if (mid && l == L / 2) AGZ_HIP_TRY(hipEventRecord(mid, st));
  }
  HeadArgs h{};
  h.x = d_actB; h.conv = d_head_conv; h.bn = d_head_bn; h.Wp = d_Wp; h.bp = d_bp; h.W1 = d_W1; h.b1 = d_b1; h.W2 = d_W2;
  h.b2 = d_b2; h.policy = policy_dev; h.value = value_dev;
  h.H = H; h.W = W; h.HW = HW; h.Wp_ = Wp; h.HpWp = Hp * Wp; h.Kp = Kp; h.A = conf.ActionSpace; h.FC = conf.FC;
  heads_spread_range(h, plan.heads_nb, B, b0, nb, st);
  AGZ_HIP_TRY(hipGetLastError());
  return AGZ_OK;
}

int agz_net::forward_packed(int B, float* policy_dev, float* value_dev) {
  AGZ_REQUIRE(committed, AGZ_E_STATE, "agz_net: infer before agz_net_commit");
  AGZ_REQUIRE(B >= 1 && B <= max_batch, AGZ_E_INVALID, "agz_net: batch %d exceeds allocated %d", B, max_batch);
  ConvArgs a{};
  a.M = B * HW; a.HW = HW; a.W = W; a.Wp = Wp; a.HpWp = Hp * Wp;
  a.x = d_act_in; a.w = d_w_init; a.ep = d_ep_init; a.y = d_actA;
  a.Cin_p = Fp; a.Cout_p = Kp; a.Ntot = Kp;
  const FwdPlan plan = fwd_plan(B);
  const bool half_init = plan.half_init, half_dual = plan.half_dual, latency = plan.latency, heads_spread = plan.heads_spread, split_ok = plan.split_ok;
  float** wsp = latency ? &d_ws : nullptr;
  int compute_mode = this->compute_mode;
  if (compute_mode == AGZ_COMPUTE_AUTO) compute_mode = !d_u2_dual.empty() ? AGZ_COMPUTE_WINO_H2 : AGZ_COMPUTE_BF16X3;
  const bool use_h2 = split_ok && compute_mode == AGZ_COMPUTE_FP16X2;
  const bool wino_ok = split_ok && compute_mode == AGZ_COMPUTE_WINO;
  const bool wino_h2_ok = split_ok && compute_mode == AGZ_COMPUTE_WINO_H2;
  if (wino_h2_ok && d_ep_init_h2) a.ep = d_ep_init_h2;
  if (use_h2 && (size_t)B > amax_cap) {
    AGZ_HIP_TRY(hipStreamSynchronize(ctx->stream));
    if (d_amax) hipFree(d_amax);
    d_amax = nullptr; amax_cap = 0;
    AGZ_HIP_TRY(hipMalloc(&d_amax, (size_t)B * sizeof(unsigned)));
    amax_cap = (size_t)B;
  }
  bool lat_h2 = latency && cfg == 0 && this->compute_mode != AGZ_COMPUTE_F32_MFMA && conf.SharedLayers > 0 &&
                (int)d_lat_w2.size() == conf.SharedLayers && agz::conv_lat_ok(Kp, Kp, Wp) && ceil_div(HW, agz::LAT_ROWS) * (Kp / 8) <= 256;
  for (int l = 0; lat_h2 && l < conf.SharedLayers; l++) lat_h2 = d_lat_w2[l] != nullptr;
  const int in_groups = ceil_div(HW, agz::LAT_IN_PIX), in_words = in_groups * (Kp / 64);
  const bool lat_in = lat_h2 && Fp == 32 && Kp % 64 == 0 && in_words <= 256 && d_w_init_t;
  if (lat_h2 && lat_wmax_cap < B) {
    AGZ_HIP_TRY(hipStreamSynchronize(ctx->stream));
    for (auto& p2 : d_lat_wmax) { if (p2) hipFree(p2); p2 = nullptr; }
    lat_wmax_cap = 0;
    for (auto& p2 : d_lat_wmax) AGZ_HIP_TRY(hipMalloc(&p2, (size_t)B * 256 * sizeof(float)));
    lat_wmax_cap = B;
  }
  int rc;
  bool amax0_done = false;
  if (lat_in) {
    agz::LatInArgs li{};
    li.x = d_act_in; li.w = d_w_init_t; li.ep = reinterpret_cast<const float2*>(d_ep_init); li.t = d_lat_tin[0]; li.y = d_actA; li.words = d_lat_wmax[1];
    li.B = B; li.H = H; li.W = W; li.Hp = Hp; li.Wp = Wp; li.Cout_p = Kp; li.groups_per_board = in_groups;
    ProfScope ps(ctx, AGZ_PROF_CONV_INIT);
    hipLaunchKernelGGL(agz::lat_input_kernel, dim3(Kp / 64, B * in_groups), dim3(256), 0, ctx->stream, li);
    rc = AGZ_OK;
  }
  else if (split_ok && compute_mode != AGZ_COMPUTE_F32_MFMA && d_w3_init && Kp % 128 == 0 &&
      (size_t)B * Hp * Wp * Fp * sizeof(float) < ((size_t)1 << 32)) {
    a.n_ntiles = ceil_div(a.Ntot, 128); a.n_mtiles = ceil_div(a.M, 128);
    a.splits = 1; a.per = 0; a.ws = nullptr; a.raw = 0;
    ProfScope ps(ctx, AGZ_PROF_CONV_INIT);
    if (wino_h2_ok && d_amax && amax_cap >= (size_t)B) {
      AGZ_HIP_TRY(hipMemsetAsync(d_amax, 0, (size_t)B * sizeof(unsigned), ctx->stream));
      a.amax_out = d_amax; amax0_done = true;
    }
    hipLaunchKernelGGL((conv3x3_x3_kernel<false>), dim3(a.n_mtiles * a.n_ntiles), dim3(256), 0, ctx->stream, a, d_w3_init);
    a.amax_out = nullptr;
    rc = AGZ_OK;
  }
  else if (cfg != 0) rc = launch_conv<4, 1, 1, false>(ctx, a, wsp, &ws_cap);
  else if (half_init) rc = launch_conv<2, 2, 1, false>(ctx, a, wsp, &ws_cap);
  else rc = launch_conv<2, 2, 2, false>(ctx, a, wsp, &ws_cap);
  if (rc != AGZ_OK) return rc;
  float* cur = d_actA;
  float* nxt = d_actB;
  bool tower_done = false;
  if (!tower_done && wino_h2_ok) {
    AGZ_REQUIRE((int)d_u2_dual.size() == conf.SharedLayers, AGZ_E_STATE, "agz_net: Winograd fp16x2 weights not built");
    const bool wide = plan.wino_wide;
    const H2Tower tw = wino_h2_tower(B);
    const int chunk = tw.chunk, ns = tw.ns;
    const size_t v_elems = tw.v_elems, m_elems = tw.m_elems, wm_board = tw.wm_board;
    const bool chained = tw.chained;
    {
      bool amax_moved = false;
      const int rr = wino_h2_reserve(B, tw, &amax_moved);
      if (rr != AGZ_OK) return rr;
      if (amax_moved) amax0_done = false;
    }
    float* d_wave_max = reinterpret_cast<float*>(d_amax + (size_t)(conf.SharedLayers + 1) * B);
    if (!amax0_done)
// ... 352 lines not shown
        for (int ci = 0; ci < K; ci++) for (int t = 0; t < 9; t++)
          wt[((size_t)t * 2 * Kp + nidx) * Kp + ci] = w.v[((size_t)o * K + ci) * 9 + t];
      }
    }
    std::vector<float> ep((size_t)hw * Kp * 4, 0.f);
    for (int p = 0; p < hw; p++) for (int o = 0; o < K; o++) {
      float* e = &ep[((size_t)p * Kp + o) * 4];
      fold(bi, o, n->params[pi + 1], n->params[pi + 2], p, &e[0], &e[1]);
      fold(bi + 1, o, n->params[pi + 4], n->params[pi + 5], p, &e[2], &e[3]);
    }
    int r;
    if ((r = upload(&n->d_w_dual[l], wt, s)) != AGZ_OK) return r;
    if ((r = upload(&n->d_ep_dual[l], ep, s)) != AGZ_OK) return r;
    if ((int)n->h_ep_dual.size() != c.SharedLayers) n->h_ep_dual.assign(c.SharedLayers, std::vector<float>());
    n->h_ep_dual[l] = ep;
    if (n->cfg == 0) {
      const int NC16 = Kp / 16, Ntot = 2 * Kp;
      std::vector<unsigned short> w3((size_t)9 * NC16 * 3 * Ntot * 16);
      for (int t = 0; t < 9; t++) for (int nn = 0; nn < Ntot; nn++) for (int ci = 0; ci < Kp; ci++) {
        float v = wt[((size_t)t * Ntot + nn) * Kp + ci];
        uint32_t u, hu, mu, lu; memcpy(&u, &v, 4);
        hu = u & 0xffff0000u; float hf; memcpy(&hf, &hu, 4);
        float r1 = v - hf; uint32_t ru; memcpy(&ru, &r1, 4);
        mu = ru & 0xffff0000u; float mf; memcpy(&mf, &mu, 4);
        float r2 = r1 - mf; memcpy(&lu, &r2, 4);
        size_t base = (((size_t)((ci / 16) * 9 + t) * 3) * Ntot + nn) * 16 + (ci % 16);
        w3[base] = (unsigned short)(hu >> 16);
        w3[base + (size_t)Ntot * 16] = (unsigned short)(mu >> 16);
        w3[base + (size_t)2 * Ntot * 16] = (unsigned short)(lu >> 16);
      }
      {
        const int NC32 = Kp / 32;
        float wmax = 0.f;
        for (float v : wt) wmax = std::max(wmax, std::fabs(v));
        int ex = 0;
        if (wmax > 0.f) std::frexp(wmax, &ex);
        const float sb = wmax > 0.f ? std::ldexp(1.0f, 14 - ex) : 1.0f;
        n->w_unscale[l] = 1.0f / sb;
        std::vector<_Float16> w2((size_t)9 * NC32 * 2 * Ntot * 32);
        for (int t = 0; t < 9; t++) for (int nn = 0; nn < Ntot; nn++) for (int ci = 0; ci < Kp; ci++) {
          float xs = wt[((size_t)t * Ntot + nn) * Kp + ci] * sb;
          _Float16 hi = (_Float16)xs;
          _Float16 lo = (_Float16)(xs - (float)hi);
          size_t base = (((size_t)((ci / 32) * 9 + t) * 2) * Ntot + nn) * 32 + (ci % 32);
          w2[base] = hi;
          w2[base + (size_t)Ntot * 32] = lo;
        }
        if (n->d_w2_dual[l]) { hipFree(n->d_w2_dual[l]); n->d_w2_dual[l] = nullptr; }
        AGZ_HIP_TRY(hipMalloc(&n->d_w2_dual[l], w2.size() * 2));
        AGZ_HIP_TRY(hipMemcpyAsync(n->d_w2_dual[l], w2.data(), w2.size() * 2, hipMemcpyHostToDevice, s));
        AGZ_HIP_TRY(hipStreamSynchronize(s));
      }
      if (n->d_w3_dual[l]) { hipFree(n->d_w3_dual[l]); n->d_w3_dual[l] = nullptr; }
      AGZ_HIP_TRY(hipMalloc(&n->d_w3_dual[l], w3.size() * 2));
      AGZ_HIP_TRY(hipMemcpyAsync(n->d_w3_dual[l], w3.data(), w3.size() * 2, hipMemcpyHostToDevice, s));
      AGZ_HIP_TRY(hipStreamSynchronize(s));
      if (agz::conv_lat_ok(Kp, Kp, n->Wp)) {
        if ((int)n->d_lat_w2.size() != c.SharedLayers) {
          n->d_lat_w2.assign(c.SharedLayers, nullptr); n->d_lat_tin.assign(c.SharedLayers, nullptr); n->d_lat_colun.assign(c.SharedLayers, nullptr);
        }
        std::vector<float> tin(Kp, 1.0f), colun(Ntot, 1.0f), su(Ntot, 1.0f), rmax(Kp, 0.f), cmax(Ntot, 0.f);
        for (int t = 0; t < 9; t++) for (int nn = 0; nn < Ntot; nn++) for (int ci = 0; ci < Kp; ci++)
          rmax[ci] = std::max(rmax[ci], std::fabs(wt[((size_t)t * Ntot + nn) * Kp + ci]));
        for (int ci = 0; ci < Kp; ci++)
          if (rmax[ci] > 0.f && std::isfinite(rmax[ci])) { int ex = 0; std::frexp(rmax[ci], &ex); tin[ci] = std::ldexp(1.0f, std::max(-100, std::min(100, ex - 1))); }
        for (int t = 0; t < 9; t++) for (int nn = 0; nn < Ntot; nn++) for (int ci = 0; ci < Kp; ci++)
          cmax[nn] = std::max(cmax[nn], std::fabs(wt[((size_t)t * Ntot + nn) * Kp + ci] / tin[ci]));
        for (int nn = 0; nn < Ntot; nn++)
          if (cmax[nn] > 0.f && std::isfinite(cmax[nn])) { int ex = 0; std::frexp(cmax[nn], &ex); su[nn] = std::ldexp(1.0f, 14 - ex); colun[nn] = 1.0f / su[nn]; }
        std::vector<_Float16> l2((size_t)9 * (Kp / 32) * 2 * Ntot * 32);
        for (int t = 0; t < 9; t++) for (int nn = 0; nn < Ntot; nn++) for (int ci = 0; ci < Kp; ci++) {
          const float xs = wt[((size_t)t * Ntot + nn) * Kp + ci] / tin[ci] * su[nn];
          const _Float16 hi = (_Float16)xs;
          const _Float16 lo = (_Float16)(xs - (float)hi);
          const size_t base = (((size_t)((ci / 32) * 9 + t) * 2) * Ntot + nn) * 32 + (ci % 32);
          l2[base] = hi;
          l2[base + (size_t)Ntot * 32] = lo;
        }
        if (n->d_lat_w2[l]) { hipFree(n->d_lat_w2[l]); n->d_lat_w2[l] = nullptr; }
        AGZ_HIP_TRY(hipMalloc(&n->d_lat_w2[l], l2.size() * 2));
        AGZ_HIP_TRY(hipMemcpyAsync(n->d_lat_w2[l], l2.data(), l2.size() * 2, hipMemcpyHostToDevice, s));
        int r2;
        if ((r2 = upload(&n->d_lat_tin[l], tin, s)) != AGZ_OK) return r2;
        if ((r2 = upload(&n->d_lat_colun[l], colun, s)) != AGZ_OK) return r2;
        AGZ_HIP_TRY(hipStreamSynchronize(s));
      }
    }
    pi += 6; bi += 2;
  }
  {
    std::vector<float> hc((size_t)3 * Kp, 0.f), hb((size_t)3 * hw * 2, 0.f);
    const Param& pw = n->params[pi];
    for (int o = 0; o < 2; o++) for (int ci = 0; ci < K; ci++) hc[(size_t)o * Kp + ci] = pw.v[(size_t)o * K + ci];
    for (int o = 0; o < 2; o++) for (int p = 0; p < hw; p++)
      fold(bi, o, n->params[pi + 1], n->params[pi + 2], p, &hb[((size_t)o * hw + p) * 2], &hb[((size_t)o * hw + p) * 2 + 1]);
    pi += 3; bi++;
    int r;
    if ((r = upload(&n->d_Wp, n->params[pi].v, s)) != AGZ_OK) return r;
    if ((r = upload(&n->d_bp, n->params[pi + 1].v, s)) != AGZ_OK) return r;
    pi += 2;
    const Param& vw = n->params[pi];
    for (int ci = 0; ci < K; ci++) hc[(size_t)2 * Kp + ci] = vw.v[ci];
    for (int p = 0; p < hw; p++)
      fold(bi, 0, n->params[pi + 1], n->params[pi + 2], p, &hb[((size_t)2 * hw + p) * 2], &hb[((size_t)2 * hw + p) * 2 + 1]);
    pi += 3; bi++;
    if ((r = upload(&n->d_W1, n->params[pi].v, s)) != AGZ_OK) return r;
    if ((r = upload(&n->d_b1, n->params[pi + 1].v, s)) != AGZ_OK) return r;
    pi += 2;
    if ((r = upload(&n->d_W2, n->params[pi].v, s)) != AGZ_OK) return r;
    if ((r = upload(&n->d_b2, n->params[pi + 1].v, s)) != AGZ_OK) return r;
    pi += 2;
    if ((r = upload(&n->d_head_conv, hc, s)) != AGZ_OK) return r;
    if ((r = upload(&n->d_head_bn, hb, s)) != AGZ_OK) return r;
    (void)A; (void)FCn;
  }
  n->committed = true;
  for (auto& p : n->d_u2_dual) if (p) hipFree(p);
  n->d_u2_dual.clear();
  for (auto& p : n->d_u2_tin) if (p) hipFree(p);
  n->d_u2_tin.clear();
  for (auto& p : n->d_u2_colun) if (p) hipFree(p);
  n->d_u2_colun.clear();
  n->free_u2c();
  for (auto& p : n->d_ep_h2) if (p) hipFree(p);
  n->d_ep_h2.clear();
  if (n->d_ep_init_h2) { hipFree(n->d_ep_init_h2); n->d_ep_init_h2 = nullptr; }
  if (n->compute_mode == AGZ_COMPUTE_WINO && n->cfg == 0) return n->build_wino_weights();
  if ((n->compute_mode == AGZ_COMPUTE_WINO_H2 || n->compute_mode == AGZ_COMPUTE_AUTO) && n->cfg == 0) return n->build_wino_h2_weights();
  return AGZ_OK;
}

int agz_wino_h2_tile(int H, int W) { return agz::wino_h2_pick_tm(H, W); }

int agz_wino_h2_chained(int H, int W, int K) {
  static const int form_env = [] { const char* e = getenv("AGZ_WINO_H2_FORM"); return e ? atoi(e) : -1; }();
  const int Kp = agz::round_up(K, 32);
  return form_env != 0 && agz::wino_h2c_ok(H, W, agz::wino_h2_pick_tm(H, W), Kp) ? 1 : 0;
}

int agz_net_set_wino_h2_form(agz_net* n, int form) {
  AGZ_REQUIRE(n, AGZ_E_INVALID, "agz_net_set_wino_h2_form: null net");
  AGZ_REQUIRE(form >= -1 && form <= 2, AGZ_E_INVALID, "agz_net_set_wino_h2_form: form %d (want -1, 0 or 1)", form);
  n->wino_form = form;
  return AGZ_OK;
}

int agz_net_min_same_batch(agz_net* n, int k, int G, int* batch) {
  AGZ_REQUIRE(n && batch && k >= 1 && G >= k, AGZ_E_INVALID, "agz_net_min_same_batch: bad argument");
  AGZ_REQUIRE(n->committed, AGZ_E_STATE, "agz_net_min_same_batch: commit the net first");
  *batch = n->min_same_batch(k, G);
  return AGZ_OK;
}

int agz_net_set_wino_h2_gemm(agz_net* n, int variant) {
  AGZ_REQUIRE(n, AGZ_E_INVALID, "agz_net_set_wino_h2_gemm: null net");
  AGZ_REQUIRE(((variant & 63) <= 2 && (variant >> 6) <= 1) || ((variant & 15) == 2 && (variant >> 4) <= 3), AGZ_E_INVALID, "agz_net_set_wino_h2_gemm: variant %d (want 0, 1, 2, + 64, or 2 + 16 * mode)", variant);
  n->wino_gemm = variant;
  return AGZ_OK;
}

int agz_wino_stages(agz_ctx* ctx, const float* x, const float* w, int B, int H, int W, int C, int N, float* V, float* M) {
  AGZ_REQUIRE(ctx && x && w && V && M, AGZ_E_INVALID, "agz_wino_stages: NULL argument");
  AGZ_REQUIRE(B >= 1 && H >= 1 && W >= 1 && C >= 16 && C % 16 == 0 && N >= 1, AGZ_E_INVALID, "agz_wino_stages: bad shape");
  AGZ_HIP_TRY(hipSetDevice(ctx->device));
  const int Hp = H + 2, Wp = W + 2;
  std::vector<float> xp((size_t)B * Hp * Wp * C, 0.f);
  for (int b = 0; b < B; b++) for (int h = 0; h < H; h++)
    memcpy(&xp[(((size_t)b * Hp + h + 1) * Wp + 1) * C], &x[((size_t)b * H + h) * W * C], (size_t)W * C * sizeof(float));
  std::vector<unsigned short> u3;
  agz::wino_build_u3(u3, N, C, [&](int n, int ci, int tap) -> double { return (double)w[((size_t)n * C + ci) * 9 + tap]; });
  agz::WinoArgs a{};
  a.B = B; a.H = H; a.W = W; a.Hp = Hp; a.Wp = Wp; a.C = C; a.Cout_p = N; a.Ntot = N;
  const size_t T = (size_t)B * agz::ceil_div(H, 4) * agz::ceil_div(W, 4);
  AGZ_REQUIRE((size_t)36 * T * C * 4 < ((size_t)1 << 32), AGZ_E_UNSUPPORTED, "agz_wino_stages: V above 4 GiB");
  float *dx = nullptr, *dV = nullptr, *dM = nullptr;
  unsigned short* dU = nullptr;
  int rc = AGZ_OK;
  if (hipMalloc(&dx, xp.size() * 4) != hipSuccess || hipMalloc(&dV, (size_t)36 * T * C * 4) != hipSuccess ||
      hipMalloc(&dM, (size_t)36 * T * N * 4) != hipSuccess || hipMalloc(&dU, u3.size() * 2) != hipSuccess) {
    agz::set_error("agz_wino_stages: out of device memory");
    rc = AGZ_E_NOMEM;
  } else {
    hipStream_t s = ctx->stream;
    bool ok = hipMemcpyAsync(dx, xp.data(), xp.size() * 4, hipMemcpyHostToDevice, s) == hipSuccess &&
              hipMemcpyAsync(dU, u3.data(), u3.size() * 2, hipMemcpyHostToDevice, s) == hipSuccess;
    a.x = dx; a.V = dV; a.U3 = dU; a.Mb = dM;
    if (ok) agz::wino_launch(ctx, a, agz::WINO_IN | agz::WINO_GEMM);
    ok = ok && hipGetLastError() == hipSuccess &&
         hipMemcpyAsync(V, dV, (size_t)36 * T * C * 4, hipMemcpyDeviceToHost, s) == hipSuccess &&
         hipMemcpyAsync(M, dM, (size_t)36 * T * N * 4, hipMemcpyDeviceToHost, s) == hipSuccess && hipStreamSynchronize(s) == hipSuccess;
    if (!ok) { agz::set_error("agz_wino_stages: HIP failure: %s", hipGetErrorString(hipGetLastError())); rc = AGZ_E_HIP; }
  }
  if (dx) hipFree(dx);
  if (dV) hipFree(dV);
  if (dM) hipFree(dM);
  if (dU) hipFree(dU);
  return rc;
}

int agz_net_set_compute_mode(agz_net* n, int mode) {
  AGZ_REQUIRE(n, AGZ_E_INVALID, "agz_net_set_compute_mode: NULL net");
  const int base = mode & ~AGZ_COMPUTE_FORCE;
  AGZ_REQUIRE(base == AGZ_COMPUTE_F32_MFMA || base == AGZ_COMPUTE_BF16X3 || base == AGZ_COMPUTE_FP16X2 || base == AGZ_COMPUTE_WINO || base == AGZ_COMPUTE_AUTO ||
                  base == AGZ_COMPUTE_WINO_H2,
              AGZ_E_INVALID, "agz_net_set_compute_mode: unknown mode %d", mode);
  n->compute_mode = base;
  n->compute_force = (mode & AGZ_COMPUTE_FORCE) != 0;
  if (base == AGZ_COMPUTE_WINO && n->committed && n->cfg == 0 && n->d_u3_dual.empty()) return n->build_wino_weights();
  if ((base == AGZ_COMPUTE_WINO_H2 || base == AGZ_COMPUTE_AUTO) && n->committed && n->cfg == 0 && n->d_u2_dual.empty()) return n->build_wino_h2_weights();
  return AGZ_OK;
}

int agz_net_set_tower_queues(agz_net* n, int queues) {
  AGZ_REQUIRE(n && queues >= 0 && queues <= 2, AGZ_E_INVALID, "agz_net_set_tower_queues: queues must be 0 (auto), 1 or 2");
  n->tower_queues = queues;
  return AGZ_OK;
}

int agz_net_set_latency_mode(agz_net* n, int on) {
  AGZ_REQUIRE(n, AGZ_E_INVALID, "agz_net_set_latency_mode: NULL net");
  n->latency_mode = on != 0;
  return AGZ_OK;
}

int agz_net_infer_dev(agz_net* n, const float* planes_dev, int B, float* policy_dev, float* value_dev) {
  AGZ_REQUIRE(n && planes_dev && policy_dev && value_dev && B >= 1, AGZ_E_INVALID, "agz_net_infer_dev: bad argument");
  AGZ_HIP_TRY(hipSetDevice(n->ctx->device));
  return n->forward_dev(planes_dev, B, policy_dev, value_dev);
}

int agz_net_infer(agz_net* n, const float* planes, int B, float* policy, float* value) {
  AGZ_REQUIRE(n && planes && policy && value && B >= 1, AGZ_E_INVALID, "agz_net_infer: bad argument");
  AGZ_REQUIRE(n->committed, AGZ_E_STATE, "agz_net_infer: call agz_net_commit first");
  AGZ_HIP_TRY(hipSetDevice(n->ctx->device));
  int r = n->ensure_batch(B);
  if (r != AGZ_OK) return r;
  hipStream_t s = n->ctx->stream;
  size_t per = (size_t)n->conf.Features * n->HW;
  AGZ_HIP_TRY(hipMemcpyAsync(n->d_planes, planes, (size_t)B * per * sizeof(float), hipMemcpyHostToDevice, s));
  r = n->forward_dev(n->d_planes, B, n->d_policy, n->d_value);
  if (r != AGZ_OK) return r;
  AGZ_HIP_TRY(hipMemcpyAsync(policy, n->d_policy, (size_t)B * n->conf.ActionSpace * sizeof(float), hipMemcpyDeviceToHost, s));
  AGZ_HIP_TRY(hipMemcpyAsync(value, n->d_value, (size_t)B * sizeof(float), hipMemcpyDeviceToHost, s));
  AGZ_HIP_TRY(hipStreamSynchronize(s));
  return AGZ_OK;
}

int agz_net_save(const agz_net* n, const char* path) {
  AGZ_REQUIRE(n && path, AGZ_E_INVALID, "agz_net_save: NULL argument");
  FILE* f = fopen(path, "wb");
  AGZ_REQUIRE(f, AGZ_E_INVALID, "agz_net_save: cannot open %s", path);
  bool ok = fwrite("AGZNET01", 1, 8, f) == 8 && fwrite(&n->conf, sizeof(agz_net_conf), 1, f) == 1;
  uint64_t np = n->params.size();
  ok = ok && fwrite(&np, 8, 1, f) == 1;
  for (const Param& p : n->params) {
    uint64_t cnt = p.v.size();
    ok = ok && fwrite(&cnt, 8, 1, f) == 1 && fwrite(p.v.data(), 4, cnt, f) == cnt;
  }
  for (const BNStats& b : n->bn) {
    uint64_t C = b.mean.size();
    ok = ok && fwrite(&C, 8, 1, f) == 1 && fwrite(b.mean.data(), 4, C, f) == C && fwrite(b.var.data(), 4, C, f) == C;
  }
  ok = (fclose(f) == 0) && ok;
  AGZ_REQUIRE(ok, AGZ_E_INVALID, "agz_net_save: write to %s failed", path);
  return AGZ_OK;
}

int agz_net_load(agz_net* n, const char* path) {
  AGZ_REQUIRE(n && path, AGZ_E_INVALID, "agz_net_load: NULL argument");
  FILE* f = fopen(path, "rb");
  AGZ_REQUIRE(f, AGZ_E_INVALID, "agz_net_load: cannot open %s", path);
  char magic[8];
  agz_net_conf c;
  uint64_t np = 0;
  bool ok = fread(magic, 1, 8, f) == 8 && memcmp(magic, "AGZNET01", 8) == 0 && fread(&c, sizeof(c), 1, f) == 1 && fread(&np, 8, 1, f) == 1;
  if (ok) ok = memcmp(&c, &n->conf, sizeof(c)) == 0 && np == n->params.size();
  if (!ok) { fclose(f); agz::set_error("agz_net_load: %s is not a checkpoint of this network configuration", path); return AGZ_E_INVALID; }
  for (Param& p : n->params) {
    uint64_t cnt = 0;
    ok = ok && fread(&cnt, 8, 1, f) == 1 && cnt == p.v.size() && fread(p.v.data(), 4, cnt, f) == cnt;
  }
  for (BNStats& b : n->bn) {
    uint64_t C = 0;
    ok = ok && fread(&C, 8, 1, f) == 1 && C == b.mean.size() && fread(b.mean.data(), 4, C, f) == C && fread(b.var.data(), 4, C, f) == C;
  }
  fclose(f);
  AGZ_REQUIRE(ok, AGZ_E_INVALID, "agz_net_load: %s is truncated or mismatched", path);
  n->committed = false;
  return agz_net_commit(n);
}

double agz_net_flops_per_eval(const agz_net* n) {
  if (!n) return 0;
  double K = n->conf.K, F = n->conf.Features, hw = n->HW, A = n->conf.ActionSpace, L = n->conf.SharedLayers, FCn = n->conf.FC;
  return 2 * F * K * 9 * hw + L * 2 * (2 * K * K * 9 * hw) + (2 * K * 2 * hw + 2 * 2 * hw * A) + (2 * K * hw + 2 * hw * FCn + 2 * FCn);
}

}
```

agogo_amd/csrc/net.hpp:

```cpp
#pragma once
#include <string>
#include <vector>

#include "common.hpp"

namespace agz {
struct Param {
  std::string name;
  std::vector<float> v;
  std::vector<int> ref_shape;
  int kind;
};
struct BNStats { std::vector<float> mean, var; };
int conv3x3_raw(agz_ctx* ctx, const float* x, const float* w, float* y, int B, int H, int W, int Cin_p, int Cout_p);
int conv3x3_raw_x3(agz_ctx* ctx, const float* x, const unsigned short* w3, float* y, int B, int H, int W, int Cin_p, int Cout_p);
int split_w3(agz_ctx* ctx, const float* w, unsigned short* w3, int N, int Cin_p);
inline size_t w3_elems(int N, int Cin_p) { return (size_t)9 * 3 * N * Cin_p; }
struct WinoRawScratch {
  float* V = nullptr; float* M = nullptr; void* U2 = nullptr; unsigned* words = nullptr;
  size_t v_cap = 0, m_cap = 0, u_cap = 0; int b_cap = 0;
  void* w2 = nullptr; unsigned* h2_words = nullptr;
  size_t w2_cap = 0; int h2_b_cap = 0, h2_flip = 0;
};
int conv3x3_raw_h2(agz_ctx* ctx, const float* x, const float* w, float* y, int B, int H, int W, int Cin_p, int Cout_p, WinoRawScratch* sc,
                   const unsigned* ranges = nullptr);
bool conv3x3_raw_h2_fits(int B, int H, int W, int Cin_p, int Cout_p);
int conv3x3_raw_h2_weights(agz_ctx* ctx, const float* w, int Cin_p, int Cout_p, WinoRawScratch* sc, const void** w2, const unsigned** w_amax);
struct RawWeights { void* img = nullptr; unsigned* words = nullptr; size_t cap = 0; };
int conv3x3_raw_h2_weights_to(agz_ctx* ctx, hipStream_t st, const float* w, int Cin_p, int Cout_p, RawWeights* out);
int conv3x3_raw_wino_h2_weights_to(agz_ctx* ctx, hipStream_t st, const float* w, int H, int W, int Cin_p, int Cout_p, RawWeights* out);
void raw_weights_free(RawWeights* rw);
int conv3x3_raw_wino_h2(agz_ctx* ctx, const float* x, const float* w, float* y, int B, int H, int W, int Cin_p, int Cout_p, WinoRawScratch* sc,
                        const unsigned* ranges = nullptr, const RawWeights* pre = nullptr);
bool conv3x3_raw_wino_h2_fits(int B, int H, int W, int Cin_p, int Cout_p);
void wino_raw_scratch_free(WinoRawScratch* sc);
struct HeadArgs;
}

struct agz_net {
  agz_ctx* ctx = nullptr;
  agz_net_conf conf{};
  std::vector<agz::Param> params;
  std::vector<agz::BNStats> bn;
  bool committed = false;

  int H = 0, W = 0, HW = 0, Hp = 0, Wp = 0;
  int Kp = 0;
  int Fp = 32;
  int cfg = 0;

  float* d_w_init = nullptr;
  float* d_w_init_t = nullptr;
  float* d_ep_init = nullptr;
  unsigned short* d_w3_init = nullptr;
  std::vector<float*> d_w_dual;
  std::vector<float*> d_ep_dual;
  std::vector<unsigned short*> d_w3_dual;
  std::vector<_Float16*> d_w2_dual;
  std::vector<float> w_unscale;
  std::vector<unsigned short*> d_u3_dual;
  std::vector<_Float16*> d_u2_dual;
  std::vector<float> u_unscale;
  std::vector<float*> d_u2_tin;
  std::vector<float*> d_u2_colun;
  std::vector<_Float16*> d_u2c_dual;
  std::vector<float> wino_g1, wino_g0;
  int wino_gemm = 0;
  int wino_form = -1;
  void free_u2c() { for (auto& p : d_u2c_dual) if (p) hipFree(p); d_u2c_dual.clear(); wino_g1.clear(); wino_g0.clear(); }
  int build_wino_h2_weights();
  int wino_tm = 4;
  size_t wino_v_cap = 0;
  float* d_wV = nullptr;
  float* d_wM = nullptr;
  int wino_chunk_cap = 0;
  int build_wino_weights();
  unsigned* d_amax = nullptr;
  size_t amax_cap = 0;
  int compute_mode = AGZ_COMPUTE_F32_MFMA;
  bool compute_force = false;
  float* d_head_conv = nullptr;
  float* d_head_bn = nullptr;
  float* d_Wp = nullptr;
  float* d_bp = nullptr;
  float* d_W1 = nullptr;
  float* d_b1 = nullptr;
  float* d_W2 = nullptr;
  float* d_b2 = nullptr;

  int max_batch = 0;
  float* d_act_in = nullptr;
  float* d_actA = nullptr;
  float* d_actB = nullptr;
  float* d_planes = nullptr;
  float* d_policy = nullptr;
  float* d_value = nullptr;
  float* d_ws = nullptr;
  std::vector<std::vector<float>> h_ep_dual;
  std::vector<float> h_ep_init;
  std::vector<float*> d_ep_h2;
  float* d_ep_init_h2 = nullptr;
  std::vector<_Float16*> d_lat_w2;
  std::vector<float*> d_lat_tin, d_lat_colun;
  float* d_lat_wmax[2] = {nullptr, nullptr};
  int lat_wmax_cap = 0;
  size_t ws_cap = 0;
  float* d_hs = nullptr;
  size_t hs_cap = 0;
  int tower_queues = 0;
  bool latency_mode = true;

  int ensure_batch(int B);
  void free_device();
  int forward_dev(const float* planes_dev, int B, float* policy_dev, float* value_dev);
  int forward_packed(int B, float* policy_dev, float* value_dev);
  struct FwdPlan { bool half_init, half_dual, small, forced_split, latency, heads_spread, split_ok, heads_nb, wino_wide; };
  FwdPlan fwd_plan(int B) const;
  int min_same_batch(int n, int G) const;
  struct H2Tower { int npos, tpb, chunk, ns, n_scr, form_want; bool chained; size_t v_elems, m_elems, wm_board; };
  H2Tower wino_h2_tower(int B) const;
  int wino_h2_reserve(int B, const H2Tower& t, bool* amax_moved);
  void wino_h2c_block(int l, int B, int b0, int ci, const H2Tower& t, hipStream_t st, float* cur, float* nxt);
  void heads_spread_range(agz::HeadArgs h, bool nb4, int B, int b0, int nb, hipStream_t st);
  bool half_ok(int B) const;
  int forward_half_reserve(int B);
  int forward_half(int B, int half, hipStream_t st, float* policy_dev, float* value_dev, hipEvent_t mid);
};
```

include/agz_debug.h:

```cpp
#ifndef AGZ_DEBUG_H
#define AGZ_DEBUG_H

#include "agz.h"

#ifdef __cplusplus
extern "C" {
#endif

#define AGZ_PROF_CONV 0
#define AGZ_PROF_HEADS 1
#define AGZ_PROF_SELECT 2
#define AGZ_PROF_EXPAND 3
#define AGZ_PROF_MOVE 4
#define AGZ_PROF_CONV_INIT 5
#define AGZ_PROF_WINO_IN 6
#define AGZ_PROF_WINO_GEMM 7
#define AGZ_PROF_WINO_OUT 8
#define AGZ_PROF_NCLASS 9
int agz_ctx_prof_enable(agz_ctx* ctx, int enable);
int agz_ctx_prof_read(agz_ctx* ctx, int klass, int64_t* launches, double* total_ms);
int agz_ctx_prof_set_stride(agz_ctx* ctx, int klass, int stride);

int agz_wino_stages(agz_ctx* ctx, const float* x, const float* w, int B, int H, int W, int C, int N, float* V, float* M);

int agz_wino_h2_tile(int H, int W);

int agz_wino_h2_chained(int H, int W, int K);

int agz_net_set_wino_h2_form(agz_net* net, int form);

int agz_net_set_wino_h2_gemm(agz_net* net, int variant);

int agz_arena_set_prep_compact(agz_arena* arena, int on);
int agz_arena_last_prep_batch(agz_arena* arena, int* boards, int* roots);

int agz_arena_set_split(agz_arena* arena, int mode);
int agz_arena_split_steps(agz_arena* arena, int64_t* split, int64_t* joined, int* last_split);

int agz_trainer_set_dma_forward(agz_trainer* t, int on);

int agz_net_min_same_batch(agz_net* net, int n, int G, int* batch);

#define AGZ_CNT_PATHMAX 15
int agz_arena_debug_counter(agz_arena* arena, int which, int64_t* value);

int agz_arena_pool_capacity(agz_arena* arena, int* nodes_per_pool, int* grows);

int agz_comm_debug_fail_slice(agz_comm* comm, int k);

int agz_comm_debug_fail_layer(agz_comm* comm, int layer);

#ifdef __cplusplus
}
#endif
#endif
```

Baseline: 42570.

## Skip dead Winograd tile rows in fp16x2 GEMM for partial edge tiles

When the board size leaves the last tile row or column partly outside the image, some transform positions hold rows that contribute nothing to the output. The input transform now stores those positions in a compacted row layout. The GEMM drops A-tile loads and MFMA sub-blocks for rows past the live count, and the output kernels read with the matching remapped offsets. This cuts MFMA work and memory traffic for those positions, at the cost of more complex indexing, a few extra eligibility conditions, and a bit to disable it.

```diff
diff --git a/agogo_amd/capi.py b/agogo_amd/capi.py
--- a/agogo_amd/capi.py
+++ b/agogo_amd/capi.py
@@ -235,6 +235,7 @@
     sig("agz_wino_h2_tile", i32, i32, i32)
     sig("agz_net_set_wino_h2_form", i32, vp, i32)
     sig("agz_net_set_wino_h2_gemm", i32, vp, i32)
+    sig("agz_net_wino_h2_last_rows", i32, vp, C.POINTER(C.c_int), C.POINTER(C.c_int))
     sig("agz_net_min_same_batch", i32, vp, i32, i32, C.POINTER(C.c_int))
     sig("agz_arena_set_prep_compact", i32, vp, i32)
     sig("agz_arena_set_split", i32, vp, i32)
@@ -439,6 +440,11 @@
     def set_wino_h2_gemm(self, variant):
         _check(lib().agz_net_set_wino_h2_gemm(self.h, int(variant)), "agz_net_set_wino_h2_gemm")
 
+    def wino_h2_last_rows(self):
+        r, c = C.c_int(0), C.c_int(0)
+        _check(lib().agz_net_wino_h2_last_rows(self.h, C.byref(r), C.byref(c)), "agz_net_wino_h2_last_rows")
+        return r.value, c.value
+
     def min_same_batch(self, n, G):
         b = C.c_int(0)
         _check(lib().agz_net_min_same_batch(self.h, int(n), int(G), C.byref(b)), "agz_net_min_same_batch")
diff --git a/agogo_amd/csrc/conv_wino_h2.hpp b/agogo_amd/csrc/conv_wino_h2.hpp
--- a/agogo_amd/csrc/conv_wino_h2.hpp
+++ b/agogo_amd/csrc/conv_wino_h2.hpp
@@ -70,6 +70,7 @@
   float g1, g0;
   int gemm_variant;
   int temporal_stores;
+  int live_r, live_c;
   int row_pad;
 };
 __device__ __forceinline__ size_t h2_row(const WinoH2Args& h, int pos, int t) {
@@ -150,6 +151,8 @@
   const size_t word_in_row = (size_t)(c >> 5) * 32 + ((c & 31) >> 1);
   const int lane = threadIdx.x & 63;
   const size_t swap_word = (size_t)((c2 >> 6) * 4) * 32 + lane;
+  const int row_r = (h.cform && h.live_r) ? maps::rows_row(maps::ROWS_R, a.nty, a.ntx, b % (128 / a.TPB), ty, tx) : (t & 127);
+  const int row_c = (h.cform && h.live_c) ? maps::rows_row(maps::ROWS_C, a.nty, a.ntx, b % (128 / a.TPB), ty, tx) : (t & 127);
 #pragma unroll
   for (int i = 0; i < AL; i++) {
     float ox[AL], oy[AL];
@@ -164,7 +167,10 @@
         const unsigned e0 = s16[0], e1 = s16[1];
         const int NS = a.C >> 5;
         const size_t chunk0 = ((size_t)(t >> 7) * h.npos + (size_t)(i * AL + j)) * NS + (size_t)((c2 >> 6) * 4 + 2 * (lane >> 5));
-        unsigned* p0 = V2 + chunk0 * 4096 + (size_t)(t & 127) * 32 + (lane & 31);
+        const int cls = maps::rows_class(true, true, AL, i, j);
+        const int row = cls == maps::ROWS_R ? row_r : (cls == maps::ROWS_C ? row_c : (t & 127));
+        if (row < 0) continue;
+        unsigned* p0 = V2 + chunk0 * 4096 + (size_t)row * 32 + (lane & 31);
         p0[0] = e0;
         p0[4096] = e1;
         continue;
diff --git a/agogo_amd/csrc/conv_wino_h2c.hpp b/agogo_amd/csrc/conv_wino_h2c.hpp
--- a/agogo_amd/csrc/conv_wino_h2c.hpp
+++ b/agogo_amd/csrc/conv_wino_h2c.hpp
@@ -135,46 +135,60 @@
 #pragma unroll
       for (int r = 0; r < 16; r++) acc[i][j][r] = 0.f;
 
+  const int live = maps::rows_pos_live(h.live_r, h.live_c, h.tm + 2, pos);
+  const bool a_on = maps::h2c_wave_row0(wid, 128) < live;
+  const int ni = (maps::h2c_mfma_row0(wm, 0) < live ? 1 : 0) + (maps::h2c_mfma_row0(wm, 1) < live ? 1 : 0);
+  auto k_loop = [&](auto ni_c) {
+    constexpr int NI = decltype(ni_c)::value;
 #pragma nounroll
-  for (int it = 0; it < NK; it++) {
-#pragma unroll
-    for (int j = 0; j < maps::h2c_wave_instrs(128); j++)
-      __builtin_amdgcn_raw_ptr_buffer_load_lds(ar, (h2c_lds_ptr_t)(la + maps::h2c_dma_dst(0, j)), 16, (j & 1) ? vo_o : vo_e,
-                                               a_so + (maps::h2c_dma_src(0, j) - maps::h2c_dma_src(0, j & 1)), 0, 0);
-#pragma unroll
-    for (int j = 0; j < maps::h2c_wave_instrs(256); j++)
-      __builtin_amdgcn_raw_ptr_buffer_load_lds(br, (h2c_lds_ptr_t)(lb + maps::h2c_dma_dst(0, j)), 16, (j & 1) ? vo_o : vo_e,
-                                               b_so + (maps::h2c_dma_src(0, j) - maps::h2c_dma_src(0, j & 1)), 0, 0);
-    a_so += SA; b_so += b_step;
-    __syncthreads();
-#pragma unroll
-    for (int ks = 0; ks < 2; ks++) {
-      f16x8_t A_[2][2];
-#pragma unroll
-      for (int i = 0; i < 2; i++) {
-        A_[i][0] = *reinterpret_cast<const f16x8_t*>(lds + maps::h2c_frag(wm * 64 + i * 32, lane, 0, ks));
-        A_[i][1] = *reinterpret_cast<const f16x8_t*>(lds + maps::h2c_frag(wm * 64 + i * 32, lane, 1, ks));
-      }
-#pragma unroll
-      for (int j = 0; j < 4; j++) {
-        const f16x8_t b0 = *reinterpret_cast<const f16x8_t*>(lds + SA + maps::h2c_frag(wn * 128 + j * 32, lane, 0, ks));
-        const f16x8_t b1 = *reinterpret_cast<const f16x8_t*>(lds + SA + maps::h2c_frag(wn * 128 + j * 32, lane, 1, ks));
-#pragma unroll
-        for (int i = 0; i < 2; i++) {
-          acc[i][j] = __builtin_amdgcn_mfma_f32_32x32x16_f16(A_[i][1], b0, acc[i][j], 0, 0, 0);
-          acc[i][j] = __builtin_amdgcn_mfma_f32_32x32x16_f16(A_[i][0], b1, acc[i][j], 0, 0, 0);
-          acc[i][j] = __builtin_amdgcn_mfma_f32_32x32x16_f16(A_[i][0], b0, acc[i][j], 0, 0, 0);
+    for (int it = 0; it < NK; it++) {
+      if (a_on) {
+#pragma unroll
+        for (int j = 0; j < maps::h2c_wave_instrs(128); j++)
+          __builtin_amdgcn_raw_ptr_buffer_load_lds(ar, (h2c_lds_ptr_t)(la + maps::h2c_dma_dst(0, j)), 16, (j & 1) ? vo_o : vo_e,
+                                                   a_so + (maps::h2c_dma_src(0, j) - maps::h2c_dma_src(0, j & 1)), 0, 0);
+      }
+#pragma unroll
+      for (int j = 0; j < maps::h2c_wave_instrs(256); j++)
+        __builtin_amdgcn_raw_ptr_buffer_load_lds(br, (h2c_lds_ptr_t)(lb + maps::h2c_dma_dst(0, j)), 16, (j & 1) ? vo_o : vo_e,
+                                                 b_so + (maps::h2c_dma_src(0, j) - maps::h2c_dma_src(0, j & 1)), 0, 0);
+      a_so += SA; b_so += b_step;
+      __syncthreads();
+      if (NI > 0) {
+#pragma unroll
+        for (int ks = 0; ks < 2; ks++) {
+          f16x8_t A_[2][2];
+#pragma unroll
+          for (int i = 0; i < NI; i++) {
+            A_[i][0] = *reinterpret_cast<const f16x8_t*>(lds + maps::h2c_frag(maps::h2c_mfma_row0(wm, i), lane, 0, ks));
+            A_[i][1] = *reinterpret_cast<const f16x8_t*>(lds + maps::h2c_frag(maps::h2c_mfma_row0(wm, i), lane, 1, ks));
+          }
+#pragma unroll
+          for (int j = 0; j < 4; j++) {
+            const f16x8_t b0 = *reinterpret_cast<const f16x8_t*>(lds + SA + maps::h2c_frag(wn * 128 + j * 32, lane, 0, ks));
+            const f16x8_t b1 = *reinterpret_cast<const f16x8_t*>(lds + SA + maps::h2c_frag(wn * 128 + j * 32, lane, 1, ks));
+#pragma unroll
+            for (int i = 0; i < NI; i++) {
+              acc[i][j] = __builtin_amdgcn_mfma_f32_32x32x16_f16(A_[i][1], b0, acc[i][j], 0, 0, 0);
+              acc[i][j] = __builtin_amdgcn_mfma_f32_32x32x16_f16(A_[i][0], b1, acc[i][j], 0, 0, 0);
+              acc[i][j] = __builtin_amdgcn_mfma_f32_32x32x16_f16(A_[i][0], b0, acc[i][j], 0, 0, 0);
+            }
+          }
         }
       }
-    }
-    __syncthreads();
-  }
+      __syncthreads();
+    }
+  };
+  if (ni == 2) k_loop(std::integral_constant<int, 2>{});
+  else if (ni == 1) k_loop(std::integral_constant<int, 1>{});
+  else k_loop(std::integral_constant<int, 0>{});
 
   float* mbase = a.Mb + maps::mc_index(m_tile, h.npos, pos, a.Ntot >> 6, n_tile * 4 + wn * 2, wm * 64, lane);
 #pragma unroll
   for (int qq = 0; qq < 2; qq++)
 #pragma unroll
-    for (int i = 0; i < 2; i++)
+    for (int i = 0; i < 2; i++) {
+      if (i >= ni) continue;
 #pragma unroll
       for (int r = 0; r < 16; r++) {
         const unsigned x0 = __float_as_uint(acc[i][2 * qq][r]), x1 = __float_as_uint(acc[i][2 * qq + 1][r]);
@@ -189,6 +203,7 @@
           d[maps::mc_index(0, 0, 0, 0, 0, 4, 0)] = __uint_as_float(w1);
         }
       }
+    }
 }
 
 
@@ -395,6 +410,16 @@
   const __amdgpu_buffer_rsrc_t mr = h2_rsrc(a.Mb + ((size_t)(t0 >> 7) * h.npos * NS + s) * 8192);
   const unsigned m_lane = (unsigned)(((tc & 127) * 64 + pr * 4) * 4);
   const unsigned m_pos = (unsigned)NS * 32768u;
+  const int bpt = 128 / a.TPB;
+  auto m_row = [&](int cls) -> unsigned {
+    const int r = maps::rows_row(cls, a.nty, a.ntx, b % bpt, ty, tx);
+    return r < 0 ? 0x80000000u : (unsigned)((r * 64 + pr * 4) * 4);
+  };
+  const unsigned m_lane_r = h.live_r ? m_row(maps::ROWS_R) : m_lane, m_lane_c = h.live_c ? m_row(maps::ROWS_C) : m_lane;
+  auto m_voff = [&](int xi, int nu) -> unsigned {
+    const int cls = maps::rows_class(true, true, AL, xi, nu);
+    return cls == maps::ROWS_R ? m_lane_r : (cls == maps::ROWS_C ? m_lane_c : m_lane);
+  };
   float Y[TM][TM][4];
 #pragma unroll
   for (int k = 0; k < TM; k++)
@@ -404,12 +429,12 @@
       for (int e = 0; e < 4; e++) Y[k][l][e] = 0.f;
   float4 m[2][AL];
 #pragma unroll
-  for (int xi = 0; xi < AL; xi++) m[0][xi] = h2_ldf4(mr, m_lane, (unsigned)(xi * AL) * m_pos);
+  for (int xi = 0; xi < AL; xi++) m[0][xi] = h2_ldf4(mr, m_voff(xi, 0), (unsigned)(xi * AL) * m_pos);
 #pragma unroll
   for (int nu = 0; nu < AL; nu++) {
     if (nu + 1 < AL) {
 #pragma unroll
-      for (int xi = 0; xi < AL; xi++) m[(nu + 1) & 1][xi] = h2_ldf4(mr, m_lane, (unsigned)(xi * AL + nu + 1) * m_pos);
+      for (int xi = 0; xi < AL; xi++) m[(nu + 1) & 1][xi] = h2_ldf4(mr, m_voff(xi, nu + 1), (unsigned)(xi * AL + nu + 1) * m_pos);
     }
     float mm[4][AL], oo[4][TM];
 #pragma unroll
@@ -603,6 +628,21 @@
   const unsigned m_lane = (unsigned)((tl * 64 + pr * 4) * 4);
   const unsigned v_lane = (unsigned)((((tid >> 6) * 4) * 128) + lane * 4);
   const unsigned e_pix = (unsigned)a.Cout_p * 16u;
+  constexpr unsigned OOB = 0x80000000u;
+  const unsigned gr_r = h.live_r ? (unsigned)(bpg * maps::rows_per_board(maps::ROWS_R, a.nty, a.ntx)) : 16u;
+  const unsigned gr_c = h.live_c ? (unsigned)(bpg * maps::rows_per_board(maps::ROWS_C, a.nty, a.ntx)) : 16u;
+  auto m_row = [&](int cls) -> unsigned {
+    const int r = maps::rows_row(cls, a.nty, a.ntx, bl, ty, tx);
+    return r < 0 ? OOB : (unsigned)((r * 64 + pr * 4) * 4);
+  };
+  auto v_row = [&](int cls, int k) -> unsigned {
+    const int tv = (tid >> 6) * 4 + 2 * k + (lane >> 5), ttv = tv % a.TPB;
+    const int r = maps::rows_row(cls, a.nty, a.ntx, tv / a.TPB, ttv / a.ntx, ttv % a.ntx);
+    return r < 0 ? OOB : (unsigned)(r * 128 + (lane & 31) * 4);
+  };
+  const unsigned m_lane_r = h.live_r ? m_row(maps::ROWS_R) : m_lane, m_lane_c = h.live_c ? m_row(maps::ROWS_C) : m_lane;
+  const unsigned v0_r = h.live_r ? v_row(maps::ROWS_R, 0) : v_lane, v1_r = h.live_r ? v_row(maps::ROWS_R, 1) : v_lane + 256u;
+  const unsigned v0_c = h.live_c ? v_row(maps::ROWS_C, 0) : v_lane, v1_c = h.live_c ? v_row(maps::ROWS_C, 1) : v_lane + 256u;
   float* const ybase = ys + ((size_t)bl * PH * PW + (size_t)(TM * ty) * PW + TM * tx) * 32 + 2 * pr;
   unsigned okmask = 0;
 #pragma unroll
@@ -611,14 +651,22 @@
     for (int l = 0; l < TM; l++) okmask |= (TM * ty + k < a.H && TM * tx + l < a.W) ? 1u << (k * TM + l) : 0u;
   const __amdgpu_buffer_rsrc_t er = h2_rsrc(a.ep);
   float4 m[NPRE][AL];
-  auto m_soff = [&](int g, int s, int pos) -> unsigned { return (unsigned)((((g >> 3) * h.npos + pos) * NS + s)) * 32768u + (unsigned)(g & 7) * 4096u; };
+  auto m_soff = [&](int g, int s, int xi, int nu) -> unsigned {
+    const int cls = maps::rows_class(true, true, AL, xi, nu);
+    const unsigned gr = cls == maps::ROWS_R ? gr_r : (cls == maps::ROWS_C ? gr_c : 16u);
+    return (unsigned)((((g >> 3) * h.npos + xi * AL + nu) * NS + s)) * 32768u + (unsigned)(g & 7) * (gr * 256u);
+  };
+  auto m_voff = [&](int xi, int nu) -> unsigned {
+    const int cls = maps::rows_class(true, true, AL, xi, nu);
+    return cls == maps::ROWS_R ? m_lane_r : (cls == maps::ROWS_C ? m_lane_c : m_lane);
+  };
   int item = blockIdx.x;
   {
     const int g = __builtin_amdgcn_readfirstlane(item / NS), s = __builtin_amdgcn_readfirstlane(item - (item / NS) * NS);
 #pragma unroll
     for (int nu = 0; nu < NPRE; nu++)
 #pragma unroll
-      for (int xi = 0; xi < AL; xi++) m[nu][xi] = h2_ldf4<MAUX>(mr, m_lane, m_soff(g, s, xi * AL + nu));
+      for (int xi = 0; xi < AL; xi++) m[nu][xi] = h2_ldf4<MAUX>(mr, m_voff(xi, nu), m_soff(g, s, xi, nu));
   }
   __syncthreads();
   for (; item < n_items; item += gridDim.x) {
@@ -643,7 +691,7 @@
       }
       if (nu + NPRE < AL) {
 #pragma unroll
-        for (int xi = 0; xi < AL; xi++) m[nu % NPRE][xi] = h2_ldf4<MAUX>(mr, m_lane, m_soff(g, s, xi * AL + nu + NPRE));
+        for (int xi = 0; xi < AL; xi++) m[nu % NPRE][xi] = h2_ldf4<MAUX>(mr, m_voff(xi, nu + NPRE), m_soff(g, s, xi, nu + NPRE));
       }
       wino_atv_p<TM>(c0, o0);
       wino_atv_p<TM>(c1, o1);
@@ -719,10 +767,11 @@
 #pragma unroll
       for (int nu = 0; nu < NPRE; nu++)
 #pragma unroll
-        for (int xi = 0; xi < AL; xi++) m[nu][xi] = h2_ldf4<MAUX>(mr, m_lane, m_soff(g2, s2, xi * AL + nu));
+        for (int xi = 0; xi < AL; xi++) m[nu][xi] = h2_ldf4<MAUX>(mr, m_voff(xi, nu), m_soff(g2, s2, xi, nu));
     }
     __builtin_amdgcn_sched_barrier(0);
-    const unsigned v_base = (unsigned)((((g >> 3) * h.npos) * NS + s)) * 16384u + (unsigned)(g & 7) * 2048u;
+    const unsigned v_base = (unsigned)((((g >> 3) * h.npos) * NS + s)) * 16384u;
+    const unsigned v_g = (unsigned)(g & 7) * 2048u, v_g_r = (unsigned)(g & 7) * (gr_r * 128u), v_g_c = (unsigned)(g & 7) * (gr_c * 128u);
     const unsigned v_pos = (unsigned)NS * 16384u;
     const float* yr = ybase;
     asm volatile("" : "+v"(yr));
@@ -758,8 +807,10 @@
           const unsigned e0 = s16[0], e1 = s16[1];
           const auto s32 = __builtin_amdgcn_permlane32_swap(e0, e1, false, false);
           const unsigned w0 = s32[0], w1 = s32[1];
-          __builtin_amdgcn_raw_buffer_store_b32(w0, vr, v_lane, v_base + (unsigned)(i * AL + j) * v_pos, VAUX);
-          __builtin_amdgcn_raw_buffer_store_b32(w1, vr, v_lane + 256u, v_base + (unsigned)(i * AL + j) * v_pos, VAUX);
+          const int cls = maps::rows_class(true, true, AL, i, j);
+          const unsigned v_so = v_base + (cls == maps::ROWS_R ? v_g_r : (cls == maps::ROWS_C ? v_g_c : v_g)) + (unsigned)(i * AL + j) * v_pos;
+          __builtin_amdgcn_raw_buffer_store_b32(w0, vr, cls == maps::ROWS_R ? v0_r : (cls == maps::ROWS_C ? v0_c : v_lane), v_so, VAUX);
+          __builtin_amdgcn_raw_buffer_store_b32(w1, vr, cls == maps::ROWS_R ? v1_r : (cls == maps::ROWS_C ? v1_c : v_lane + 256u), v_so, VAUX);
         }
       }
       __builtin_amdgcn_sched_barrier(0);
@@ -799,6 +850,30 @@
   a.n_mtiles = ceil_div(a.T, 128); a.n_ntiles = ceil_div(a.Ntot, 128);
   h.in_swap = 1; h.cform = 1; h.wm_per_board = 0;
 }
+constexpr int WINO_H2_GEMM_DEFAULT = 1;
+static inline int wino_h2c_gemm_variant(const WinoH2Args& h) { return h.gemm_variant > 0 ? h.gemm_variant : WINO_H2_GEMM_DEFAULT; }
+static inline bool wino_h2c_dma_ok(const WinoH2Args& h) {
+  return wino_h2_rows(h.npos, (size_t)h.w.T) * h.w.C * 4 < ((size_t)1 << 31) && (size_t)h.npos * h.w.C * h.w.Ntot * 4 < ((size_t)1 << 31);
+}
+static inline bool wino_h2c_fits31(const WinoH2Args& h) { return wino_h2_rows(h.npos, (size_t)h.w.T) * h.w.Ntot * 4 < ((size_t)1 << 31); }
+static bool wino_h2c_oip_ready(agz_ctx* ctx) {
+  if (!(ctx->func_attr_state & 2u)) {
+    const bool ok = hipFuncSetAttribute(reinterpret_cast<const void*>(&wino_oip_h2c_kernel<5>), hipFuncAttributeMaxDynamicSharedMemorySize, 80 * 1024) == hipSuccess &&
+                    hipFuncSetAttribute(reinterpret_cast<const void*>(&wino_oip_h2c_kernel<4>), hipFuncAttributeMaxDynamicSharedMemorySize, 80 * 1024) == hipSuccess;
+    if (!ok) (void)hipGetLastError();
+    ctx->func_attr_state |= 2u | (ok ? 1u : 0u);
+  }
+  return (ctx->func_attr_state & 1u) != 0;
+}
+static void wino_h2c_rows(agz_ctx* ctx, WinoH2Args& h, int oi_variant, bool keep_all) {
+  wino_h2c_geometry(h);
+  h.live_r = h.live_c = 0;
+  const int gemm = wino_h2c_gemm_variant(h) & 15;
+  const maps::WinoRows g = maps::wino_rows(h.w.H, h.w.W, h.tm);
+  if (keep_all || gemm != 1 || oi_variant != 4 || !wino_h2c_dma_ok(h) || !wino_h2c_fits31(h) || !maps::rows_short_ok(g) || !wino_h2c_oip_ready(ctx)) return;
+  h.live_r = g.dead_y ? maps::rows_slot_live(g, maps::ROWS_R) : 0;
+  h.live_c = g.dead_x ? maps::rows_slot_live(g, maps::ROWS_C) : 0;
+}
 static void wino_h2c_in(agz_ctx* ctx, WinoH2Args& h, hipStream_t st) {
   wino_h2c_geometry(h);
   h.fuse_prev = 0; h.amax_self = const_cast<unsigned*>(h.amax_in);
@@ -807,13 +882,12 @@
   if (h.tm == 5) hipLaunchKernelGGL(wino_in_h2_kernel<5>, dim3((unsigned)((n_in + 255) / 256)), dim3(256), 0, st, h);
   else hipLaunchKernelGGL(wino_in_h2_kernel<4>, dim3((unsigned)((n_in + 255) / 256)), dim3(256), 0, st, h);
 }
-constexpr int WINO_H2_GEMM_DEFAULT = 1;
 static void wino_h2c_gemm(agz_ctx* ctx, WinoH2Args& h, hipStream_t st) {
   wino_h2c_geometry(h);
   ProfScopeOn ps(ctx, AGZ_PROF_WINO_GEMM, st == ctx->stream.raw());
   const dim3 g(h.npos * h.w.n_mtiles * (h.w.Ntot >> 8));
-  const bool dma_ok = wino_h2_rows(h.npos, (size_t)h.w.T) * h.w.C * 4 < ((size_t)1 << 31) && (size_t)h.npos * h.w.C * h.w.Ntot * 4 < ((size_t)1 << 31);
-  const int variant_all = h.gemm_variant > 0 ? h.gemm_variant : WINO_H2_GEMM_DEFAULT;
+  const bool dma_ok = wino_h2c_dma_ok(h);
+  const int variant_all = wino_h2c_gemm_variant(h);
   const int variant = variant_all & 15, mode = (variant_all >> 4) & 3;
   const int n_slabs = h.w.Ntot >> 7;
   if (variant == 2 && dma_ok && (h.w.C >> 5) == 8 && h.w.Ntot % 256 == 0 && ctx->num_cus / 8 >= n_slabs) {
@@ -848,14 +922,8 @@
   const WinoArgs& a = h.w;
   const dim3 g((unsigned)ceil_div(a.T, 16), (unsigned)(a.C >> 5));
   const size_t shm = last ? 0 : (size_t)(16 / a.TPB) * a.H * a.W * 32 * sizeof(float);
-  const bool fits31 = wino_h2_rows(h.npos, (size_t)a.T) * a.Ntot * 4 < ((size_t)1 << 31);
-  if (variant == 4 && !last && fits31 && !(ctx->func_attr_state & 2u)) {
-    const bool ok = hipFuncSetAttribute(reinterpret_cast<const void*>(&wino_oip_h2c_kernel<5>), hipFuncAttributeMaxDynamicSharedMemorySize, 80 * 1024) == hipSuccess &&
-                    hipFuncSetAttribute(reinterpret_cast<const void*>(&wino_oip_h2c_kernel<4>), hipFuncAttributeMaxDynamicSharedMemorySize, 80 * 1024) == hipSuccess;
-    if (!ok) (void)hipGetLastError();
-    ctx->func_attr_state |= 2u | (ok ? 1u : 0u);
-  }
-  if (variant == 4 && !last && fits31 && (ctx->func_attr_state & 1u)) {
+  const bool fits31 = wino_h2c_fits31(h);
+  if (variant == 4 && !last && fits31 && wino_h2c_oip_ready(ctx)) {
     const size_t shp = (size_t)(16 / a.TPB) * (h.tm * a.nty + 2) * (h.tm * a.ntx + 2) * 32 * sizeof(float);
     const int items = ceil_div(a.T, 16) * (a.C >> 5);
     const dim3 gp((unsigned)std::min(items, 2 * ctx->num_cus));
diff --git a/agogo_amd/csrc/gemm_maps.hpp b/agogo_amd/csrc/gemm_maps.hpp
--- a/agogo_amd/csrc/gemm_maps.hpp
+++ b/agogo_amd/csrc/gemm_maps.hpp
@@ -28,6 +28,43 @@
   return ((((size_t)m_tile * npos + pos) * (size_t)n_slices + (size_t)slice) * 128 + (size_t)row) * 64 + (size_t)col;
 }
 
+AGZ_MAPS_HD constexpr int h2c_wave_row0(int wid, int stage_rows) { return wid * (stage_rows / 4); }
+AGZ_MAPS_HD constexpr int h2c_mfma_row0(int wm, int i) { return wm * 64 + i * 32; }
+
+enum { ROWS_FULL = 0, ROWS_R = 1, ROWS_C = 2 };
+struct WinoRows { int TM, AL, nty, ntx, TPB, bpt; bool dead_y, dead_x; };
+AGZ_MAPS_HD constexpr WinoRows wino_rows(int H, int W, int TM) {
+  const int nty = (H + TM - 1) / TM, ntx = (W + TM - 1) / TM;
+  return WinoRows{TM, TM + 2, nty, ntx, nty * ntx, 128 / (nty * ntx), TM * nty > H, TM * ntx > W};
+}
+AGZ_MAPS_HD constexpr int rows_class(bool dead_y, bool dead_x, int AL, int xi, int nu) {
+  return xi == AL - 1 ? (dead_y ? ROWS_R : ROWS_FULL) : ((dead_x && nu == AL - 1) ? ROWS_C : ROWS_FULL);
+}
+AGZ_MAPS_HD constexpr int rows_per_board(int cls, int nty, int ntx) {
+  return cls == ROWS_R ? nty * ntx - ntx : (cls == ROWS_C ? nty * ntx - nty : nty * ntx);
+}
+AGZ_MAPS_HD constexpr int rows_local(int cls, int nty, int ntx, int ty, int tx) {
+  return cls == ROWS_R ? (ty < nty - 1 ? ty * ntx + tx : -1) : (cls == ROWS_C ? (tx < ntx - 1 ? ty * (ntx - 1) + tx : -1) : ty * ntx + tx);
+}
+AGZ_MAPS_HD constexpr int rows_row(int cls, int nty, int ntx, int bs, int ty, int tx) {
+  return rows_local(cls, nty, ntx, ty, tx) < 0 ? -1 : bs * rows_per_board(cls, nty, ntx) + rows_local(cls, nty, ntx, ty, tx);
+}
+AGZ_MAPS_HD constexpr int rows_slot_live(const WinoRows& g, int cls) { return g.bpt * rows_per_board(cls, g.nty, g.ntx); }
+AGZ_MAPS_HD constexpr bool rows_live_ok(int live) { return live == 32 || live == 64 || live == 96; }
+AGZ_MAPS_HD constexpr bool rows_short_ok(const WinoRows& g) {
+  return 128 % g.TPB == 0 && (g.dead_y || g.dead_x) && (!g.dead_y || rows_live_ok(rows_slot_live(g, ROWS_R))) &&
+         (!g.dead_x || rows_live_ok(rows_slot_live(g, ROWS_C)));
+}
+AGZ_MAPS_HD constexpr int rows_pos_live(int live_r, int live_c, int AL, int pos) {
+  return pos / AL == AL - 1 ? (live_r ? live_r : 128) : ((live_c && pos % AL == AL - 1) ? live_c : 128);
+}
+AGZ_MAPS_HD constexpr int rows_stored_per_board(const WinoRows& g) {
+  int n = 0;
+  for (int xi = 0; xi < g.AL; xi++)
+    for (int nu = 0; nu < g.AL; nu++) n += rows_per_board(rows_class(g.dead_y, g.dead_x, g.AL, xi, nu), g.nty, g.ntx);
+  return n;
+}
+
 constexpr int H2P_D = 10, H2P_R = 16, H2P_NK = 8;
 AGZ_MAPS_HD constexpr unsigned h2p_v_base(int pos, int hm, int npos) {
   return (unsigned)(((hm >> 1) * npos + pos) * (H2P_NK * 16384) + (hm & 1) * 8192);
diff --git a/agogo_amd/csrc/net.hip b/agogo_amd/csrc/net.hip
--- a/agogo_amd/csrc/net.hip
+++ b/agogo_amd/csrc/net.hip
@@ -1123,12 +1123,14 @@
     static const int gemm_env = [] {
       const char* e = getenv("AGZ_WINO_H2_GEMM");
       const int v = e ? atoi(e) : 0;
-      if (v == 0 || (((v & 63) == 1 || (v & 63) == 2) && (v >> 6) <= 1)) return v;
-      fprintf(stderr, "libagz: AGZ_WINO_H2_GEMM=%s ignored (want 1 or 2, optionally + 64)\n", e);
+      if (v == 0 || (((v & 63) == 1 || (v & 63) == 2) && (v >> 6) <= 3)) return v;
+      fprintf(stderr, "libagz: AGZ_WINO_H2_GEMM=%s ignored (want 1 or 2, optionally + 64 and / or + 128)\n", e);
       return 0;
     }();
     const int gv = wino_gemm > 0 ? wino_gemm : gemm_env;
     hh.gemm_variant = gv & 63; hh.temporal_stores = (gv >> 6) & 1;
+    agz::wino_h2c_rows(ctx, hh, t.form_want == 1 ? 1 : 4, ((gv >> 7) & 1) != 0);
+    wino_live_r = hh.live_r; wino_live_c = hh.live_c;
   }
   if (l == 0) agz::wino_h2c_in(ctx, hh, st);
   agz::wino_h2c_gemm(ctx, hh, st);
@@ -1787,9 +1789,15 @@
   return AGZ_OK;
 }
 
+int agz_net_wino_h2_last_rows(agz_net* n, int* live_r, int* live_c) {
+  AGZ_REQUIRE(n && live_r && live_c, AGZ_E_INVALID, "agz_net_wino_h2_last_rows: null argument");
+  *live_r = n->wino_live_r; *live_c = n->wino_live_c;
+  return AGZ_OK;
+}
+
 int agz_net_set_wino_h2_gemm(agz_net* n, int variant) {
   AGZ_REQUIRE(n, AGZ_E_INVALID, "agz_net_set_wino_h2_gemm: null net");
-  AGZ_REQUIRE(((variant & 63) <= 2 && (variant >> 6) <= 1) || ((variant & 15) == 2 && (variant >> 4) <= 3), AGZ_E_INVALID, "agz_net_set_wino_h2_gemm: variant %d (want 0, 1, 2, + 64, or 2 + 16 * mode)", variant);
+  AGZ_REQUIRE(((variant & 63) <= 2 && (variant >> 6) <= 3) || ((variant & 15) == 2 && (variant >> 4) <= 3), AGZ_E_INVALID, "agz_net_set_wino_h2_gemm: variant %d (want 0, 1, 2, + 64, + 128, or 2 + 16 * mode)", variant);
   n->wino_gemm = variant;
   return AGZ_OK;
 }
diff --git a/agogo_amd/csrc/net.hpp b/agogo_amd/csrc/net.hpp
--- a/agogo_amd/csrc/net.hpp
+++ b/agogo_amd/csrc/net.hpp
@@ -66,6 +66,7 @@
   std::vector<_Float16*> d_u2c_dual;
   std::vector<float> wino_g1, wino_g0;
   int wino_gemm = 0;
+  int wino_live_r = 0, wino_live_c = 0;
   int wino_form = -1;
   void free_u2c() { for (auto& p : d_u2c_dual) if (p) hipFree(p); d_u2c_dual.clear(); wino_g1.clear(); wino_g0.clear(); }
   int build_wino_h2_weights();
diff --git a/include/agz_debug.h b/include/agz_debug.h
--- a/include/agz_debug.h
+++ b/include/agz_debug.h
@@ -31,6 +31,8 @@
 
 int agz_net_set_wino_h2_gemm(agz_net* net, int variant);
 
+int agz_net_wino_h2_last_rows(agz_net* net, int* live_r, int* live_c);
+
 int agz_arena_set_prep_compact(agz_arena* arena, int on);
 int agz_arena_last_prep_batch(agz_arena* arena, int* boards, int* roots);
 
```

Measured after the change: 43760, median of 6. +2.8%, better.
